# wendongbi/Bridged-GNN

Hardware: AMD Instinct MI355X
Metric: aggregated_edges_per_sec_ktgnn_fwd (higher is better)
Workload: dtype f32; 1 GPU; C4 synthetic bridged graph (local) N=1000000 E'=20991058, 2-layer KT-GNN eval fwd F=128 hidden=128 C=2; parallelism=single, execution=eager launches

## Files before the change

### bridged_gnn_amd/_lib.py

```python
import ctypes as C
import os

import torch

_HERE = os.path.dirname(os.path.abspath(__file__))
SO_PATH = os.path.join(_HERE, "csrc", "libbgnn_hip.so")
_lib = None

_P, _I64, _I32, _F32, _SZ, _INT = C.c_void_p, C.c_int64, C.c_int32, C.c_float, C.c_size_t, C.c_int

SIGNATURES = {
    "bgnn_version": (_INT, []),
    "bgnn_source_hash": (C.c_char_p, []),
    "bgnn_error_string": (C.c_char_p, [_INT]),
    "bgnn_csr_workspace_bytes": (_SZ, [_I64, _I64]),
    "bgnn_build_dst_csr": (_INT, [_P, _I64, _I64, _INT, _P, _P, _P, _P, _P, _SZ, _P]),
    "bgnn_domain_sums_f64": (_INT, [_P, _I64, _I32, _I64, _P, _P, _P]),
    "bgnn_domain_sums_workspace_bytes": (_SZ, [_I32]),
    "bgnn_domain_sums_ws_f64": (_INT, [_P, _I64, _I32, _I64, _P, _P, _P, _SZ, _P]),
    "bgnn_domain_delta_f32": (_INT, [_P, _I32, _P, _P]),
    "bgnn_adaptedconv_transform_f32": (_INT, [_P, _I64, _I32, _I64, _P, _P, _I32, _I32, _P, _P, _P, _P,
                                               _P, _P, _P, _P, _I64, _I64, _P, _P]),
    "bgnn_adaptedconv_transform_sums_f32": (_INT, [_P, _I64, _I32, _I64, _P, _P, _I32, _I32, _P, _P, _P, _P,
                                                    _P, _P, _P, _P, _I64, _I64, _I64, _I64, _P, _P]),
    "bgnn_adaptedconv_transform_need_f32": (_INT, [_P, _I64, _I32, _I64, _P, _P, _I32, _I32, _P, _P, _P, _P,
                                                    _P, _P, _P, _P, _I64, _I64, _P, _P, _P]),
    "bgnn_classifier_stage_f32": (_INT, [_P, _I64, _I32, _I64, _P, _P, _I32, _I32, _P, _P, _P, _P, _P, _P, _P, _P, _I64, _I64,
                                          _P, _P, _I32, _INT, _P, _P, _P, _P, _P, _P]),
    "bgnn_linear_narrow_transform_f32": (_INT, [_P, _I64, _I32, _I64, _P, _P, _I32, _INT, _P, _P, _P, _P, _P, _P]),
    "bgnn_narrow_transform_finish_f32": (_INT, [_P, _I64, _P, _P, _I32, _P, _P, _P, _P, _P, _P, _I64, _P, _P]),
    "bgnn_gram_workspace_bytes": (C.c_size_t, [_I32, _I32]),
    "bgnn_gram_f32": (_INT, [_P, _I64, _I32, _P, _I64, _I32, _I64, _P, _P, C.c_size_t, _P]),
    "bgnn_transform_bwd_prep_workspace_bytes": (C.c_size_t, [_I64, _I32]),
    "bgnn_transform_bwd_prep_f32": (_INT, [_P, _I64, _I64, _I32, _P, _P, _I64, _I32, _P, _P, _P, _P, _P, _P, _I32, _I64, _P, _I64, _P, _P, C.c_size_t, _P]),
    "bgnn_bn_acc_doubles": (_I64, [_I32]),
    "bgnn_bn_relu_dropout_f32": (_INT, [_P, _I64, _I32, _I64, _P, _P, _F32, _INT, _F32, C.c_uint64, _P, _F32, _P, _P, _P, _I64, _P, _P]),
    "bgnn_bn_relu_dropout_bwd_f32": (_INT, [_P, _P, _I64, _I32, _I64, _I64, _P, _P, _P, _F32, _INT, _F32, C.c_uint64, _P, _P, _I64, _P, _P]),
    "bgnn_bn_colstats_f32": (_INT, [_P, _I64, _I32, _I64, _P, _P]),
    "bgnn_bn_apply_rows_f32": (_INT, [_P, _I64, _I32, _I64, _P, _I64, _P, _P, _F32, _INT, _F32, C.c_uint64, _P, _P, _I64, _F32, _P, _P, _P, _I64, _P]),
    "bgnn_bn_bwd_reduce_rows_f32": (_INT, [_P, _P, _I64, _I32, _I64, _I64, _P, _I64, _P, _P, _F32, _INT, _F32, C.c_uint64, _P, _P, _I64, _P, _P]),
    "bgnn_bn_bwd_apply_rows_f32": (_INT, [_P, _P, _I64, _I32, _I64, _I64, _P, _P, _I64, _P, _P, _F32, _INT, _F32, C.c_uint64, _P, _P, _I64, _P, _I64, _P]),
    "bgnn_transform_bwd_consts_f32": (_INT, [_P, _P, _P, _P, _P, _I32, _I32, _P, _P, _P, _P]),
    "bgnn_transform_bwd_finish_f32": (_INT, [_P, _P, _P, _P, _P, _P, _P, _I32, _I32, _I32, _P, _P, _P, _P, _P, _P, _P, _I64, _P]),
    "bgnn_rowdot_f32": (_INT, [_P, _I64, _I64, _I32, _P, _I64, _I32, _P, _P]),
    "bgnn_linear_f32": (_INT, [_P, _I64, _I32, _I64, _P, _P, _I32, _INT, _P, _P, _P, _I64, _P]),
    "bgnn_adaptedconv_aggregate_f32": (_INT, [_P, _P, _I64, _P, _P, _P, _P, _P, _I64, _I64, _I32, _F32,
                                               _P, _I64, _P, _P, _P, _INT, _P, _INT, _I64, _I32, _P, _P, _P]),
    "bgnn_adaptedconv_aggregate_bounded_f32": (_INT, [_P, _P, _I64, _P, _P, _P, _P, _P, _I64, _I64, _I32, _F32,
                                                       _P, _I64, _P, _P, _P, _INT, _P, _INT, _I64, _I32, _P, _P, _I64, _I32, _P]),
    "bgnn_aggregate_hub_workspace_bytes": (C.c_size_t, [_I64, _I32, _I64]),
    "bgnn_adaptedconv_aggregate_hub_f32": (_INT, [_P, _P, _I64, _P, _P, _P, _P, _P, _I64, _I32, _F32, _P, _I64, _P, _P, _INT, _P, _I32, _P,
                                                   _P, _I32, _P, _I64, _P, _P, _P, _I64, _P, _P, C.c_size_t, _P]),
    "bgnn_adaptedconv_aggregate_bwd_f32": (_INT, [_P, _P, _I64, _P, _P, _P, _P, _P, _I64, _I64, _I32, _F32,
                                                   _P, _I64, _P, _P, _I64, _P, _P, _P, _P, _P]),
    "bgnn_aggregate_bwd_pull_workspace_bytes": (C.c_size_t, [_I64, _I64, _I64]),
    "bgnn_adaptedconv_aggregate_bwd_pull_f32": (_INT, [_P, _P, _I64, _P, _P, _P, _P, _P, _P, _P, _P, _I64, _I64, _I32, _F32,
                                                        _P, _I64, _P, _P, _I64, _P, _P, _P, _P, _P, C.c_size_t, _P]),
    "bgnn_aggregate_bwd_pull_hub_workspace_bytes": (C.c_size_t, [_I64, _I64, _I64, _I64, _I64]),
    "bgnn_adaptedconv_aggregate_bwd_pull_hub_f32": (_INT, [_P, _P, _I64, _P, _P, _P, _P, _P, _P, _P, _P, _I64, _I64, _I32, _F32,
                                                            _P, _I64, _P, _P, _I64, _P, _P, _P, _P, _I32,
                                                            _P, _I64, _P, _P, _P, _I64, _P, _I64, _P, _P, _P, _I64, _P, C.c_size_t, _P]),
    "bgnn_aggregate_heads_bwd_workspace_bytes": (C.c_size_t, [_I64, _I64, _I32]),
    "bgnn_adaptedconv_aggregate_heads_bwd_f32": (_INT, [_P, _P, _P, _P, _P, _P, _P, _P, _P, _P, _I64, _I64, _I32, _I32, _F32,
                                                         _P, _P, _P, _INT, _P, _P, _P, _P, _P, C.c_size_t, _P]),
    "bgnn_aggregate_heads_bwd_hub_workspace_bytes": (C.c_size_t, [_I64, _I64, _I32, _I64, _I64]),
    "bgnn_adaptedconv_aggregate_heads_bwd_hub_f32": (_INT, [_P, _P, _P, _P, _P, _P, _P, _P, _P, _I64, _I64, _I32, _I32, _F32,
                                                             _P, _P, _P, _INT, _P, _P, _P, _P, _I32,
                                                             _P, _I64, _P, _P, _P, _I64, _P, _I64, _P, _P, _P, _I64, _P, C.c_size_t, _P]),
    "bgnn_adaptedconv_aggregate_heads_wide_f32": (_INT, [_P, _P, _I64, _P, _P, _P, _P, _P, _I64, _I32, _I32, _F32, _P, _P, _P]),
    "bgnn_aggregate_heads_wide_bwd_workspace_bytes": (C.c_size_t, [_I64, _I32, _I64]),
    "bgnn_adaptedconv_aggregate_heads_wide_bwd_f32": (_INT, [_P, _P, _I64, _P, _P, _P, _P, _P, _P, _P, _I64, _I32, _I32, _F32,
                                                              _P, _P, _P, _P, _P, _P, _P, _P, C.c_size_t, _P]),
    "bgnn_l2_normalize_rows_f32": (_INT, [_P, _I64, _I32, _F32, _P, _P]),
    "bgnn_topk_workspace_bytes": (_SZ, [_I64, _I64, _I32]),
    "bgnn_cosine_topk_f32": (_INT, [_P, _P, _I64, _I64, _I32, _I32, _INT, _P, _P, _P, _P, _SZ, _P]),
    "bgnn_mlp_pair_topk_f32": (_INT, [_P, _P, _P, _P, _P, _F32, _I64, _I64, _I32, _I32, _INT, _P, _P, _P,
                                       _P, _SZ, _P]),
    "bgnn_topk_edges_i64": (_INT, [_P, _I64, _I32, _I64, _I64, _P, _P]),
    "bgnn_topk_edges_coalesced_workspace_bytes": (_SZ, [_I64, _I32]),
    "bgnn_topk_edges_coalesced_i64": (_INT, [_P, _I64, _I32, _I64, _I64, _I64, _P, _P, _SZ, _P]),
    "bgnn_gather_rows_f32": (_INT, [_P, _I64, _I64, _P, _I64, _I32, _P, _I64, _P]),
    "bgnn_coalesce_workspace_bytes": (_SZ, [_I64]),
    "bgnn_coalesce_i64": (_INT, [_P, _I64, _I64, _P, _P, _SZ, _P]),
    "bgnn_sage_mean_aggregate_f32": (_INT, [_P, _I64, _I64, _P, _I64, _P, _P, _I64, _I32, _INT, _INT, _F32, C.c_uint64, _P,
                                             _P, _I64, _P]),
    "bgnn_sage_mean_aggregate_rows_f32": (_INT, [_P, _I64, _I64, _P, _I64, _P, _P, _I64, _I32, _INT, _INT, _F32, C.c_uint64, _P,
                                                  _P, _P, _I64, _P]),
    "bgnn_rows_segment_add_f32": (_INT, [_P, _I64, _I64, _P, _P, _P, _I64, _I32, _INT, _P, _I64, _I64, _P]),
    "bgnn_pair_mlp_workspace_bytes": (_SZ, [_I64]),
    "bgnn_pair_mlp_stats_f32": (_INT, [_P, _I64, _I64, _P, _I64, _I64, _P, _P, _I64, _F32, _P, _P, _P, _P, _SZ, _P]),
    "bgnn_pair_mlp_loss_f32": (_INT, [_P, _I64, _I64, _P, _I64, _I64, _P, _P, _P, _I64, _P, _P, _P, _P, _P, _F32, _P, _P, _P, _P,
                                       _SZ, _P]),
    "bgnn_pair_mlp_segsum_f32": (_INT, [_P, _I64, _I64, _P, _I64, _I64, _P, _P, _P, _I64, _P, _P, _P, _P, _P, _P, _F32, _P, _I64, _P]),
    "bgnn_pair_mlp_eval_f32": (_INT, [_P, _I64, _I64, _P, _I64, _I64, _P, _P, _P, _I64, _P, _P, _P, _P, _P, _P, _P, _SZ, _P]),
    "bgnn_pair_mlp_count_workspace_bytes": (_SZ, [_I64, _I64]),
    "bgnn_pair_mlp_count_f32": (_INT, [_P, _I64, _I64, _P, _I64, _I64, _P, _I64, _P, _I64, _P, _P, _P, _P, _P, _P, _P, _P, _SZ, _P]),
    "bgnn_pair_cos_loss_workspace_bytes": (_SZ, [_I64]),
    "bgnn_pair_cos_count_workspace_bytes": (_SZ, [_I64, _I64]),
    "bgnn_pair_cos_loss_f32": (_INT, [_P, _I64, _I64, _P, _I64, _I64, _P, _P, _P, _I64, _P, _P, _P, _P, _SZ, _P]),
    "bgnn_pair_cos_segsum_f32": (_INT, [_P, _I64, _I64, _P, _P, _P, _I64, _P, _I64, _P, _I64, _P]),
    "bgnn_pair_cos_count_f32": (_INT, [_P, _I64, _I64, _P, _I64, _I64, _P, _I64, _P, _I64, _P, _P, _P, _P, _SZ, _P]),
    "bgnn_sage_mean_aggregate_bwd_workspace_bytes": (_SZ, [_I64, _I32]),
    "bgnn_sage_mean_aggregate_bwd_f32": (_INT, [_P, _I64, _P, _I64, _P, _I64, _P, _P, _I64, _I32, _INT, _F32, _P, _I64, _P, _I64,
                                                 _P, _SZ, _P]),
    "bgnn_gcn_aggregate_workspace_bytes": (_SZ, [_I64, _I32]),
    "bgnn_gcn_aggregate_f32": (_INT, [_P, _I64, _I64, _P, _P, _P, _P, _I64, _I64, _I32, _INT, _F32, C.c_uint64, _P,
                                       _I32, _P, _I64, _P, _P, _I64, _P, _SZ, _P, _I64, _P]),
    "bgnn_gcn_aggregate_rows_f32": (_INT, [_P, _I64, _I64, _P, _P, _P, _P, _I64, _I64, _I32, _INT, _F32, C.c_uint64, _P,
                                            _I32, _P, _I64, _P, _P, _I64, _P, _SZ, _P, _P, _I64, _P]),
    "bgnn_gcn_aggregate_bwd_f32": (_INT, [_P, _I64, _P, _I64, _I64, _P, _P, _P, _I64, _I64, _I32, _INT, _F32,
                                           _I32, _P, _I64, _P, _P, _I64, _P, _SZ, _P, _I64, _P, _I64, _P]),
    "bgnn_step2_loss_workspace_bytes": (_SZ, [_I64, _I32]),
    "bgnn_step2_loss_f32": (_INT, [_P, _I64, _P, _I64, _P, _I64, _I64, _I32, _P, _P, _P, C.c_double, _P, _P, _SZ, _P]),
    "bgnn_step2_loss_bwd_f32": (_INT, [_P, _I64, _P, _I64, _I64, _I32, _P, _P, _P, C.c_double, _P, _P, _P, _P, _P, _I64, _P]),
    "bgnn_step2_nll_f32": (_INT, [_P, _I64, _I64, _I32, _P, _P, _P, _P, _SZ, _P]),
    "bgnn_step2_nll_bwd_f32": (_INT, [_I64, _I32, _P, _P, _P, _P, _P, _I64, _P]),
    "bgnn_step2_counts_f32": (_INT, [_P, _I64, _P, _I64, _P, _I64, _I64, _I32, _P, _P, C.c_uint64, _I32, _P, _P]),
    "bgnn_step2_auc_count_f32": (_INT, [_P, _P, _I64, _P, _P, _P, _P]),
    "bgnn_adam_chunk_elems": (_I64, []),
    "bgnn_adam_step_f32": (_INT, [_P, _I32, _P, _I64, _P, _P, _I64, C.c_double, C.c_double, C.c_double, C.c_double, _P]),
    "bgnn_quantile_workspace_bytes": (_SZ, [_I64]),
    "bgnn_quantile_f32": (_INT, [_P, _I64, C.c_double, _P, _P, _SZ, _P]),
    "bgnn_row_inv_norms_f32": (_INT, [_P, _I64, _I32, _F32, _P, _P]),
    "bgnn_edge_validity_f32": (_INT, [_P, _I64, _P, _I64, _P, _P, _P, _P, _I64, _P, _P, _P, _P, _I32, _INT, _F32, _P, _P, _I32, _P, _P, _P, _P]),
    "bgnn_edge_rule1_counts_f32": (_INT, [_P, _P, _I64, _P, _P, _P]),
}


def source_hash():
    import hashlib
    csrc = os.path.join(_HERE, "csrc")
    h = hashlib.sha256()
    for name in _HASHED_SOURCES:
        with open(os.path.join(csrc, name), "rb") as f:
            h.update(f.read())
    return h.hexdigest()[:16]


_HASHED_SOURCES = ("bgnn_api.hip", "bgnn_csr.hip", "bgnn_transform.hip", "bgnn_transform_stream.hip", "bgnn_transform_cls.hip", "bgnn_aggregate.hip", "bgnn_aggregate_bwd.hip",
                   "bgnn_aggregate_bwd_fast.hip", "bgnn_knn.hip", "bgnn_gram.hip", "bgnn_norm.hip", "bgnn_sage.hip", "bgnn_gcn.hip", "bgnn_aggregate_heads_wide.hip", "bgnn_pair_mlp.hip", "bgnn_pair_cos.hip", "bgnn_step2.hip", "bgnn_optim.hip", "bgnn_edge_filter.hip", "bgnn_common.h", "bgnn_transform_params.h", "bgnn_aggregate_bwd_params.h", os.path.join("..", "..", "include", "bgnn.h"))


def _sidecar_hash():
    try:
        with open(os.path.join(_HERE, "csrc", "libbgnn_hip.srchash")) as f:
            return f.read().strip()
    except OSError:
        return None


ABI_VERSION = 113


def _make():
    import fcntl
    import subprocess
    csrc = os.path.join(_HERE, "csrc")
    with open(os.path.join(csrc, ".build.lock"), "w") as lock:
        fcntl.flock(lock, fcntl.LOCK_EX)
        try:
            if os.path.exists(SO_PATH) and _sidecar_hash() == source_hash():
                return
            r = subprocess.run(["make", "-C", csrc, "-j4", "-s"], stdout=subprocess.PIPE, stderr=subprocess.STDOUT, text=True)
            if r.returncode != 0:
                raise RuntimeError(f"building {SO_PATH} failed (make exit code {r.returncode}):\n{r.stdout[-4000:]}")
        finally:
            fcntl.flock(lock, fcntl.LOCK_UN)


def _load():
    l = C.CDLL(SO_PATH)
    for name, (res, args) in SIGNATURES.items():
        fn = getattr(l, name)
        fn.restype, fn.argtypes = res, args
    return l


def lib():
    global _lib
    if _lib is None:
        have_hipcc = os.path.exists("/opt/rocm/bin/hipcc")
        if have_hipcc and (not os.path.exists(SO_PATH) or _sidecar_hash() != source_hash()):
            _make()
        if not os.path.exists(SO_PATH):
            raise RuntimeError(
                f"{SO_PATH} is missing: build it with `python -c 'import __graft_entry__ as g; g.build()'` "
                "(or `make -C bridged_gnn_amd/csrc`).  bridged_gnn_amd has no CPU fallback.")
        want = source_hash()
        l = _load()
        got = l.bgnn_source_hash().decode()
        if got != want:
            raise RuntimeError(
                f"{SO_PATH} was built from other sources (library {got}, tree {want}): rebuild it with "
                "`make -C bridged_gnn_amd/csrc` (a loaded library cannot be replaced inside this process)")
        if l.bgnn_version() != ABI_VERSION:
            raise RuntimeError(f"{SO_PATH} exports ABI revision {l.bgnn_version()}, this binding was written for {ABI_VERSION}")
        _lib = l
    return _lib


def check(rc, what):
    if rc != 0:
        msg = lib().bgnn_error_string(int(rc))
# ... 37 lines not shown
```

### bridged_gnn_amd/classifier_stage.py

```python
import os

import torch
import torch.nn.functional as F

from . import ops
from .ktgnn import _AggregateFn, _AggregateHeadsFn, _AggregateWideHeadsFn, _TransformPairFn, _pad_cols4, _plist


class ClassifierStage:

    def __init__(self, model):
        base = model.clf_base
        self.model, self.convs = model, (base, model.clf_target, model.clf_target)
        self.C, self.ld, self.slope = base.out_channels, ops.pad4(base.out_channels), base.negative_slope
        self.plain = not (base.root_weight or base.normalize)
        self.fused_log_softmax = ops.heads_log_softmax_supported(3, self.C)
        self.drop_caches()

    def drop_caches(self):
        self._a3_key = self._tf_key = self._tf_pack = None

    def views(self, t2s, s2t):
        ld = self.ld
        return [(t2s[:, j * ld:(j + 1) * ld], s2t[:, j * ld:(j + 1) * ld]) for j in range(3)]

    def attention(self, autograd=False):
        if autograd:
            return (torch.stack([c.a_f_t2s.weight.reshape(-1) for c in self.convs]),
                    torch.stack([c.a_f_s2t.weight.reshape(-1) for c in self.convs]))
        key = (self.convs[0]._versions(), self.convs[1]._versions())
        if self._a3_key != key:
            self._a3 = (torch.stack([c.a_f_t2s.weight.detach().reshape(-1) for c in self.convs]).contiguous(),
                        torch.stack([c.a_f_s2t.weight.detach().reshape(-1) for c in self.convs]).contiguous())
            self._a3_key = key
        return self._a3

    def finish(self, out3):
        logp = out3.view(out3.shape[0], 3, self.ld)[:, :, :self.C]
        if not self.fused_log_softmax:
            logp = F.log_softmax(logp, dim=2)
        return logp[:, 0], logp[:, 1], logp[:, 2]

    def fold_transformer(self):
        l0, bn, _, l3 = self.model.clf_transformer
        key = tuple((p.data_ptr(), p._version) for p in _plist(self.model.clf_transformer)) + \
            (bn.running_mean._version, bn.running_var._version)
        if self._tf_key != key:
            s = (bn.weight / torch.sqrt(bn.running_var + bn.eps)).detach()
            self._tf_w0 = (l0.weight.detach() * s[:, None]).float().contiguous()
            self._tf_w0t = self._tf_w0.t().contiguous()
            self._tf_b0 = (l0.bias.detach() * s + bn.bias.detach() - bn.running_mean * s).float().contiguous()
            self._tf_key = key
            self._tf_pack = None

    def transformer_hidden_eval(self, x, mask_u8=None, want_sums=False, sums_out=None):
        self.fold_transformer()
        sums = None
        dout, din = self._tf_w0.shape
        if x.dtype == torch.float32 and x.stride(1) == 1 and ops.linear_supported(din, dout):
            if want_sums:
                sums = sums_out if sums_out is not None else torch.zeros(2 * dout + 2, dtype=torch.float64, device=x.device)
            h1 = ops.linear(x, self._tf_w0, self._tf_b0, relu=True, mask_u8=mask_u8 if want_sums else None, colsum=sums)
        elif hasattr(torch, "_addmm_activation"):
            h1 = torch._addmm_activation(self._tf_b0, x, self._tf_w0t, use_gelu=False)
        else:
            h1 = F.relu(torch.addmm(self._tf_b0, x, self._tf_w0t))
        return (h1, sums) if want_sums else h1

    def transformer_eval(self, x):
        l3 = self.model.clf_transformer[3]
        return F.linear(self.transformer_hidden_eval(x), l3.weight, l3.bias)

    def composed_target_pack(self, din_pad):
        c, l3 = self.convs[1], self.model.clf_transformer[3]
        key = (din_pad, c._versions(), l3.weight._version, l3.bias._version, l3.weight.data_ptr())
        if self._tf_pack is None or self._tf_pack[0] != key:
            W3, b3 = l3.weight.detach(), l3.bias.detach()
            hd = c.head()
            din = W3.shape[0]

            def comp_gate(g):
                g = g.reshape(-1)
                return torch.cat((W3.t() @ g[:din], W3.t() @ g[din:])), (b3 * g[:din]).sum()
            g1, c1 = comp_gate(hd["g_s2t"])
            g2, c2 = comp_gate(hd["g_t2s"])
            head = {"W_s": hd["W_s"] @ W3, "W_t": hd["W_t"] @ W3,
                    "b_s": hd["W_s"] @ b3 + (hd["b_s"] if hd["b_s"] is not None else 0),
                    "b_t": hd["W_t"] @ b3 + (hd["b_t"] if hd["b_t"] is not None else 0),
                    "g_s2t": g1, "g_t2s": g2, "gate_const": (c1, c2)}
            self._tf_pack = (key, ops.pack_transform_heads([head], din_pad))
        return self._tf_pack[1]

    def one_pass(self, x, mask_u8, sums_h, views, arena):
        if sums_h is None or x.dtype != torch.float32 or x.stride(1) != 1:
            return None
        self.fold_transformer()
        dout, din = self._tf_w0.shape
        if x.shape[1] != din or dout != 128:
            return None
        pack_t = self.composed_target_pack(ops.pad4(dout))
        pair = self.convs[0].packed(x.shape[1], self.convs[1])
        if not ops.classifier_stage_supported(x, pair, self._tf_w0, pack_t):
            return None
        n_s = 2 * ops.pad4(dout) + 2
        sums_t = arena.take(n_s) if arena is not None else torch.zeros(n_s, dtype=torch.float64, device=x.device)
        raw = ops.classifier_stage(x, mask_u8, sums_h, pair, [views[0], views[1]], self._tf_w0, self._tf_b0, sums_t, pack_t, relu=True)
        return raw, None, sums_t

    def pair_tables(self, x, mask_u8, sums_h, views):
        self.convs[0].transform(x, mask_u8, sums=sums_h, partner=self.convs[1], out=[views[0], views[1]])

    def target_stage_a(self, x, mask_u8, sums_out=None):
        self.fold_transformer()
        dout, din = self._tf_w0.shape
        pack = self.composed_target_pack(ops.pad4(dout))
        if (sums_out is not None and x.dtype == torch.float32 and x.stride(1) == 1 and x.shape[1] == din
                and ops.linear_narrow_supported(din, dout, pack) and os.environ.get("BGNN_FUSED_TARGET", "1") != "0"):
            return ops.linear_narrow_transform(x, self._tf_w0, self._tf_b0, mask_u8, sums_out, pack, relu=True), None, sums_out
        h1, sums1 = self.transformer_hidden_eval(x, mask_u8, want_sums=True, sums_out=sums_out)
        h1 = _pad_cols4(h1)
        if sums1 is None or sums1.numel() != 2 * h1.shape[1] + 2:
            sums1 = ops.domain_sums(h1, mask_u8)
        return None, h1, sums1

    def target_stage_b(self, stage_a, mask_u8, out, sums_t=None):
        raw, h1, sums_t = (*stage_a[:2], sums_t if sums_t is not None else stage_a[2])
        if raw is not None:
            ops.narrow_transform_finish(raw, mask_u8, sums_t, self.composed_target_pack(ops.pad4(self._tf_w0.shape[0])), out)
        else:
            ops.adaptedconv_transform(h1, mask_u8, None, self.composed_target_pack(h1.shape[1]), out=[out], sums=sums_t)

    def target_tables(self, x, mask_u8, out, arena=None, sums_out=None):
        if sums_out is None:
            n_s = 2 * ops.pad4(self.model.clf_transformer[0].weight.shape[0]) + 2
            sums_out = arena.take(n_s) if arena is not None else torch.zeros(n_s, dtype=torch.float64, device=x.device)
        self.target_stage_b(self.target_stage_a(x, mask_u8, sums_out), mask_u8, out)

    def eval_tables(self, x, mask_u8, sums_h, views, arena):
        a = self.one_pass(x, mask_u8, sums_h, views, arena)
        if a is not None:
            return self.target_stage_b(a, mask_u8, views[2])
        self.pair_tables(x, mask_u8, sums_h, views)
        self.target_tables(x, mask_u8, views[2], arena)

    def train_walk(self, opt_in=False):
        if ops.heads_log_softmax_supported(3, self.C) and not (opt_in and os.environ.get("BGNN_FUSED_TRAIN_HEADS", "1") == "0"):
            return "narrow"
        if ops.wide_heads_supported(3, self.C) and not (opt_in and os.environ.get("BGNN_WIDE_TRAIN_HEADS", "0") != "1"):
            return "wide"
        return None if opt_in else "convs"

    def train_tables(self, x, mask_u8, sums_x, bn, sums_of=None, mean_hook=None):
        base, target, _ = self.convs
        l0, bnm, _, l3 = self.model.clf_transformer
        xt = l3(bn(l0(x), bnm, True, 0.0)).contiguous()
        sums_t = sums_of(xt) if sums_of is not None else None
        if mean_hook is None and _TransformPairFn.supported(x, base, target):
            prm = [t for c in (base, target)
                   for t in (c.lin_s.weight, c.lin_s.bias, c.lin_t.weight, c.lin_t.bias, c.a_g_s2t.weight, c.a_g_t2s.weight)]
            tabs_x = _TransformPairFn.apply(x, mask_u8, base, target, sums_x, *prm)
        else:
            tabs_x = (*base._transform_autograd(x, mask_u8, sums_x, mean_hook), *target._transform_autograd(x, mask_u8, sums_x, mean_hook))
        return (*tabs_x, *target._transform_autograd(xt, mask_u8, sums_t, mean_hook))

    def train_aggregate(self, walk, csr, mask_u8, tables, n_rows=None):
        C = self.C
        a_t, a_s = self.attention(autograd=True)
        if walk == "convs":
            return tuple(F.log_softmax(_AggregateFn.apply(tables[2 * j], tables[2 * j + 1], a_t[j], a_s[j], csr, mask_u8, C,
                                                          c.negative_slope)[:n_rows, :C], dim=1) for j, c in enumerate(self.convs))
        fn = _AggregateHeadsFn if walk == "narrow" else _AggregateWideHeadsFn
        logp = fn.apply(csr, mask_u8, C, self.slope, a_t, a_s, *tables)[:n_rows, :, :C]
        return logp[:, 0], logp[:, 1], logp[:, 2]
```

### bridged_gnn_amd/csrc/bgnn_aggregate.hip

```cpp
#include <cstdlib>
#include "bgnn_common.h"

namespace {

struct AggParams {
  const float* h_t2s;
  const float* h_s2t;
  int64_t ldh;
  const float* a_t2s;
  const float* a_s2t;
  const int32_t* rowptr;
  const int32_t* col;
  const uint8_t* mask;
  int64_t row_begin;
  int64_t row_end;
  int32_t D;
  float slope;
  float* out;
  int64_t ldo;
  float* alpha;
  const float* ep_scale;
  const float* ep_shift;
  int ep_relu;
  unsigned int* tile_queue;
  double* colsum;
  int32_t heads;
  float* state_ms;
  int mode;
  int64_t park_begin;
  int tq_chunk;
  int tq_interleave;
  int xcd_segments;
  const int32_t* vrow_node;
  const int32_t* vrow_bounds;
  int64_t n_vrows;
  float* vout; float* vms;
  int32_t hub_threshold;
  const char* tbl_base;
  uint32_t tbl_bytes, off_t2s, off_s2t;
  int32_t gather_hint;
  uint32_t dead_off;
};

__device__ __forceinline__ float leaky(float v, float slope) { return v > 0.f ? v : v * slope; }

template <int LF, int EP, int U>
__global__ __launch_bounds__(256) void agg_kernel(AggParams p) {
  constexpr int GL = LF * EP;
  constexpr int GPW = 64 / GL;
  constexpr int RPB = 4 * GPW;
  const int lane = threadIdx.x & 63;
  const int wave = threadIdx.x >> 6;
  const int g = lane / GL;
  const int lg = lane % GL;
  const int sub = lg / LF;
  const int f0 = (lg % LF) * 4;
  const bool fvalid = f0 < p.D;

  const int64_t ntiles = ((p.row_end - p.row_begin) * p.heads + RPB - 1) / RPB;
  bgnn::XcdRange tr = bgnn::xcd_pos_range(ntiles);
  __shared__ float red[2][LF * 4 + 1];
  if (p.colsum != nullptr) {
    for (int t = threadIdx.x; t < 2 * (LF * 4 + 1); t += 256) (&red[0][0])[t] = 0.f;
    __syncthreads();
  }

  __shared__ unsigned int dyn_tile;
  const int64_t xbase = tr.begin - (blockIdx.x / 8);
  int64_t tile = tr.begin - tr.step;
  int64_t chunk_left = 0;
  const int TQ_CHUNK = p.tq_chunk;
  for (;;) {
    if (p.tile_queue != nullptr) {
      if (chunk_left == 0) {
        __syncthreads();
        if (threadIdx.x == 0) dyn_tile = atomicAdd(&p.tile_queue[blockIdx.x % 8], 1u);
        __syncthreads();
        tile = xbase + (int64_t)dyn_tile * TQ_CHUNK;
        chunk_left = TQ_CHUNK;
      } else {
        tile += 1;
      }
      --chunk_left;
    } else {
      tile += tr.step;
    }
    if (tile >= tr.end) break;
    const int64_t gt = bgnn::xcd_tile_of(tile, ntiles);
    if (gt < 0) continue;
    const int64_t i = p.row_begin * p.heads + gt * RPB + wave * GPW + g;
    const bool rvalid = i < p.row_end * p.heads;
    const int64_t ic = rvalid ? i : p.row_begin * p.heads;
    const int64_t node = ic / p.heads;
    const int head = (int)(ic - node * p.heads);
    const bool dom_s = p.mask[node] != 0;
    const float* __restrict__ H = dom_s ? p.h_t2s : p.h_s2t;
    const float* __restrict__ av = (dom_s ? p.a_t2s : p.a_s2t) + head * p.D;
    const int32_t beg = rvalid ? p.rowptr[node] : 0;
    const int32_t end = rvalid ? p.rowptr[node + 1] : 0;

    float4 a4 = make_float4(0.f, 0.f, 0.f, 0.f), hi = a4;
    if (fvalid) {
      a4.x = av[f0];
      a4.y = f0 + 1 < p.D ? av[f0 + 1] : 0.f;
      a4.z = f0 + 2 < p.D ? av[f0 + 2] : 0.f;
      a4.w = f0 + 3 < p.D ? av[f0 + 3] : 0.f;
      hi = *reinterpret_cast<const float4*>(H + ic * p.ldh + f0);
    }

    float m = -INFINITY, s = 0.f;
    float4 acc = make_float4(0.f, 0.f, 0.f, 0.f);
    if (p.mode == 2 && rvalid && sub == 0) {
      m = p.state_ms[2 * i];
      s = p.state_ms[2 * i + 1];
      if (f0 < p.ldo) acc = *reinterpret_cast<const float4*>(p.out + i * p.ldo + f0);
    }
    const int32_t deg = end - beg;
    const int32_t niter = (deg + EP * U - 1) / (EP * U);

    int32_t nid[U];
#pragma unroll
    for (int u = 0; u < U; ++u) {
      int32_t e = beg + sub + u * EP;
      nid[u] = e < end ? p.col[e] : -1;
    }
    for (int32_t it = 0; it < niter; ++it) {
      const int32_t e0 = beg + it * (EP * U) + sub;
      int32_t id[U];
      float4 v[U];
#pragma unroll
      for (int u = 0; u < U; ++u) {
        id[u] = nid[u];
        v[u] = make_float4(0.f, 0.f, 0.f, 0.f);
        if (id[u] >= 0 && fvalid) v[u] = *reinterpret_cast<const float4*>(H + ((int64_t)id[u] * p.heads + head) * p.ldh + f0);
      }
#pragma unroll
      for (int u = 0; u < U; ++u) {
        int32_t e = e0 + (U + u) * EP;
        nid[u] = e < end ? p.col[e] : -1;
      }
      float lg_[U];
      float cm = -INFINITY;
#pragma unroll
      for (int u = 0; u < U; ++u) {
        float t = a4.x * leaky(v[u].x + hi.x, p.slope);
        t = fmaf(a4.y, leaky(v[u].y + hi.y, p.slope), t);
        t = fmaf(a4.z, leaky(v[u].z + hi.z, p.slope), t);
        t = fmaf(a4.w, leaky(v[u].w + hi.w, p.slope), t);
        t = bgnn::group_sum<LF>(t);
        lg_[u] = id[u] >= 0 ? t : -INFINITY;
        cm = fmaxf(cm, lg_[u]);
      }
      if (p.alpha != nullptr && (lg % LF) == 0) {
#pragma unroll
        for (int u = 0; u < U; ++u)
          if (id[u] >= 0) p.alpha[e0 + u * EP] = lg_[u];
      }
      const float mn = fmaxf(m, cm);
      const float sc = (m == mn) ? 1.f : __expf(m - mn);
      s *= sc;
      acc.x *= sc; acc.y *= sc; acc.z *= sc; acc.w *= sc;
#pragma unroll
      for (int u = 0; u < U; ++u) {
        const float pe = (lg_[u] == -INFINITY) ? 0.f : __expf(lg_[u] - mn);
        s += pe;
        acc.x = fmaf(pe, v[u].x, acc.x);
        acc.y = fmaf(pe, v[u].y, acc.y);
        acc.z = fmaf(pe, v[u].z, acc.z);
        acc.w = fmaf(pe, v[u].w, acc.w);
      }
      m = mn;
    }

#pragma unroll
    for (int off = LF; off < GL; off <<= 1) {
      const float m2 = __shfl_xor(m, off);
      const float s2 = __shfl_xor(s, off);
      float4 b;
      b.x = __shfl_xor(acc.x, off); b.y = __shfl_xor(acc.y, off);
      b.z = __shfl_xor(acc.z, off); b.w = __shfl_xor(acc.w, off);
      const float mn = fmaxf(m, m2);
      const float c1 = (m == mn) ? 1.f : __expf(m - mn);
      const float c2 = (m2 == mn) ? 1.f : __expf(m2 - mn);
      s = s * c1 + s2 * c2;
      acc.x = acc.x * c1 + b.x * c2; acc.y = acc.y * c1 + b.y * c2;
      acc.z = acc.z * c1 + b.z * c2; acc.w = acc.w * c1 + b.w * c2;
      m = mn;
    }

    if (p.mode == 1 && node >= p.park_begin) {
      if (rvalid && sub == 0) {
        if (lg == 0) { p.state_ms[2 * i] = m; p.state_ms[2 * i + 1] = s; }
        if (f0 < p.ldo) *reinterpret_cast<float4*>(p.out + i * p.ldo + f0) = fvalid ? acc : make_float4(0.f, 0.f, 0.f, 0.f);
      }
// ... 406 lines not shown
      const int32_t j = tile - xbase, sg = j / seg_len;
      gt = (sg * 8 + xcd) * seg_len + (j - sg * seg_len);
      if (gt >= ntiles) continue;
    }
    const int32_t i0 = row0 + gt * RPB + wave * GPW + g;
    const bool rvalid = i0 < row1;
    const int32_t ic = rvalid ? i0 : row0;
    const bool dom_s = p.mask[ic] != 0;
    const int32_t beg = rvalid ? p.rowptr[ic] : 0;
    const int32_t end = rvalid ? p.rowptr[ic + 1] : 0;
    const uint32_t lbase = (dom_s ? p.off_t2s : p.off_s2t) + (uint32_t)f0c * 4u;
    const f2 a01 = dom_s ? aS01 : aT01, a23 = dom_s ? aS23 : aT23;
    const float4 hi4 = __builtin_bit_cast(float4, __builtin_amdgcn_raw_buffer_load_b128(rt, lbase + __umul24((uint32_t)ic, nstride), 0, 0));
    f2 h01 = {hi4.x, hi4.y}, h23 = {hi4.z, hi4.w};

    float m = -INFINITY, s = 0.f;
    f2 acc01 = {0.f, 0.f}, acc23 = {0.f, 0.f};
    const int32_t niter = (end - beg + U - 1) / U;
    auto issue = [&](float4 (&v)[U], uint32_t off) {
      v[0] = __builtin_bit_cast(float4, __builtin_amdgcn_raw_buffer_load_b128(rt, lbase + dpp_movu<0x00>(off), 0, 0));
      v[1] = __builtin_bit_cast(float4, __builtin_amdgcn_raw_buffer_load_b128(rt, lbase + dpp_movu<0x55>(off), 0, 0));
      v[2] = __builtin_bit_cast(float4, __builtin_amdgcn_raw_buffer_load_b128(rt, lbase + dpp_movu<0xAA>(off), 0, 0));
      v[3] = __builtin_bit_cast(float4, __builtin_amdgcn_raw_buffer_load_b128(rt, lbase + dpp_movu<0xFF>(off), 0, 0));
      asm volatile("" : "+v"(h01), "+v"(h23) : : "memory");
      __builtin_amdgcn_sched_barrier(0);
    };
    auto take_id = [&](uint32_t& id) {
      __builtin_amdgcn_sched_barrier(0);
      asm volatile("s_waitcnt vmcnt(0)" : "+v"(id), "+v"(m), "+v"(s), "+v"(acc01), "+v"(acc23) : : "memory");
    };
    auto load_id = [&](int32_t ee) {
      uint32_t id;
      const uint32_t eoff = (uint32_t)max(min(ee, end - 1), 0) * 4u;
      __builtin_amdgcn_sched_barrier(0);
      asm volatile("global_load_dword %0, %1, %2" : "=v"(id) : "v"(eoff), "s"(p.col) : "memory");
      __builtin_amdgcn_sched_barrier(0);
      return id;
    };
    auto row_off = [&](uint32_t id, bool alive) { return alive ? __umul24(id, nstride) : p.dead_off; };
    auto update = [&](const float4 (&v)[U], bool ok, int32_t e_cur) {
      float t[U];
#pragma unroll
      for (int u = 0; u < U; ++u) {
        f2 z0 = f2{v[u].x, v[u].y} + h01, z1 = f2{v[u].z, v[u].w} + h23;
        z0 = __builtin_elementwise_max(z0, z0 * sl);
        z1 = __builtin_elementwise_max(z1, z1 * sl);
        f2 q = a01 * z0;
        q = __builtin_elementwise_fma(a23, z1, q);
        t[u] = q.x + q.y;
      }
      const float rA = bfly<0xB1>(b0, t[0], t[1]), rB = bfly<0xB1>(b0, t[2], t[3]);
      float r = bfly<0x4E>(b1, rA, rB);
      r += bgnn::dpp_mov<0x124>(r);
      r += bgnn::dpp_mov<0x128>(r);
      if constexpr (LF >= 32) r += bgnn::swz_xor16(r);
      if constexpr (LF >= 64) r += __shfl_xor(r, 32);
      const float l = ok ? r : -INFINITY;
      if constexpr (ALPHA) {
        if (lg < U && ok) p.alpha[e_cur] = l;
      }
      float cm = fmaxf(l, bgnn::dpp_mov<0xB1>(l));
      cm = fmaxf(cm, bgnn::dpp_mov<0x4E>(cm));
      const float mn = fmaxf(m, cm);
      const float sc = (m == mn) ? 1.f : __expf(m - mn);
      const float pe = (l == -INFINITY) ? 0.f : __expf(l - mn);
      s = fmaf(s, sc, pe);
      const f2 sc2 = {sc, sc};
      acc01 *= sc2; acc23 *= sc2;
#define BGNN_ACC(u, w)                                               \
      {                                                              \
        acc01.x = fmaf(w, v[u].x, acc01.x); acc01.y = fmaf(w, v[u].y, acc01.y); \
        acc23.x = fmaf(w, v[u].z, acc23.x); acc23.y = fmaf(w, v[u].w, acc23.y); \
      }
#ifdef AGGF_X_NOACC
      acc01.x += pe * v[0].x + v[1].y + v[2].z + v[3].w;
#else
      { const float w = quad_bcast<0>(pe); BGNN_ACC(0, w) }
      { const float w = quad_bcast<1>(pe); BGNN_ACC(1, w) }
      { const float w = quad_bcast<2>(pe); BGNN_ACC(2, w) }
      { const float w = quad_bcast<3>(pe); BGNN_ACC(3, w) }
#endif
#undef BGNN_ACC
      m = mn;
    };
    int32_t nw = __builtin_amdgcn_readlane(niter, 0);
    if constexpr (LF <= 32) nw = max(nw, __builtin_amdgcn_readlane(niter, 32));
    if constexpr (LF <= 16) nw = max(nw, max(__builtin_amdgcn_readlane(niter, 16), __builtin_amdgcn_readlane(niter, 48)));
    int32_t e = beg + k;
    bool ok = e < end;
    uint32_t myoff = p.dead_off;
    if (nw > 0) myoff = row_off((uint32_t)p.col[max(min(e, end - 1), 0)], ok);
    for (int32_t it = 0; it < nw; ++it) {
      float4 v[U];
      issue(v, myoff);
      const int32_t e_cur = e;
      e += U;
      const bool ok2 = e < end;
      uint32_t nextid = load_id(e);
      update(v, ok, e_cur);
      ok = ok2;
      take_id(nextid);
      myoff = row_off(nextid, ok);
    }
    s += bgnn::dpp_mov<0xB1>(s);
    s += bgnn::dpp_mov<0x4E>(s);

    const float inv = 1.f / (s + 1e-16f);
    if constexpr (ALPHA) {
      if (lg < U) {
        for (int32_t e2 = beg + lg; e2 < end; e2 += 4 * U) {
          float a[4];
#pragma unroll
          for (int j = 0; j < 4; ++j) a[j] = e2 + j * U < end ? p.alpha[e2 + j * U] : 0.f;
#pragma unroll
          for (int j = 0; j < 4; ++j)
            if (e2 + j * U < end) p.alpha[e2 + j * U] = __expf(a[j] - m) * inv;
        }
      }
    }
    if (rvalid && f0 < p.ldo) {
      float4 o = make_float4(acc01.x * inv, acc01.y * inv, acc23.x * inv, acc23.y * inv);
      if (p.ep_scale != nullptr) {
        o.x = fmaf(o.x, sc4[0], sh4[0]); o.y = fmaf(o.y, sc4[1], sh4[1]);
        o.z = fmaf(o.z, sc4[2], sh4[2]); o.w = fmaf(o.w, sc4[3], sh4[3]);
      }
      if (p.ep_relu) { o.x = fmaxf(o.x, 0.f); o.y = fmaxf(o.y, 0.f); o.z = fmaxf(o.z, 0.f); o.w = fmaxf(o.w, 0.f); }
      if (!fvalid) o = make_float4(0.f, 0.f, 0.f, 0.f);
      __builtin_amdgcn_raw_buffer_store_b128(__builtin_bit_cast(u32x4_t, o), ro, __umul24((uint32_t)i0, ostride) + (uint32_t)f0 * 4u, 0, 0);
      if (p.colsum != nullptr) {
        const float ws = dom_s ? 1.f : 0.f, wt = dom_s ? 0.f : 1.f;
        const f2 ws2 = {ws, ws}, wt2 = {wt, wt}, o01 = {o.x, o.y}, o23 = {o.z, o.w};
        cs_s01 = __builtin_elementwise_fma(o01, ws2, cs_s01); cs_s23 = __builtin_elementwise_fma(o23, ws2, cs_s23);
        cs_t01 = __builtin_elementwise_fma(o01, wt2, cs_t01); cs_t23 = __builtin_elementwise_fma(o23, wt2, cs_t23);
        n_s += ws; n_t += wt;
      }
    }
  }
  if (p.colsum != nullptr) {
    unsafeAtomicAdd(&red[0][f0], cs_s01.x); unsafeAtomicAdd(&red[0][f0 + 1], cs_s01.y);
    unsafeAtomicAdd(&red[0][f0 + 2], cs_s23.x); unsafeAtomicAdd(&red[0][f0 + 3], cs_s23.y);
    unsafeAtomicAdd(&red[1][f0], cs_t01.x); unsafeAtomicAdd(&red[1][f0 + 1], cs_t01.y);
    unsafeAtomicAdd(&red[1][f0 + 2], cs_t23.x); unsafeAtomicAdd(&red[1][f0 + 3], cs_t23.y);
    if (lg == 0) { unsafeAtomicAdd(&red[0][LF * 4], n_s); unsafeAtomicAdd(&red[1][LF * 4], n_t); }
    __syncthreads();
    for (int t = threadIdx.x; t < 2 * (LF * 4 + 1); t += 256) {
      const int d = t / (LF * 4 + 1), c = t % (LF * 4 + 1);
      const double sum = (double)red[d][c];
      if (c == LF * 4) unsafeAtomicAdd(&p.colsum[2 * p.ldo + d], sum);
      else if (c < p.ldo) unsafeAtomicAdd(&p.colsum[d * p.ldo + c], sum);
    }
  }
}

template <int HEADS, int EP, int U>
__global__ __launch_bounds__(256) void agg_heads_lanes_kernel(AggParams p) {
  constexpr int GL = EP * HEADS, GPW = 64 / GL, RPB = 4 * GPW;
  const int lane = threadIdx.x & 63, wave = threadIdx.x >> 6;
  const int g = lane / GL, lg = lane % GL;
  const int sub = lg / HEADS, h = lg % HEADS;
  const bool lane_on = g < GPW;
  const int64_t ntiles = (p.row_end - p.row_begin + p.n_vrows + RPB - 1) / RPB;
  bgnn::XcdRange tr = bgnn::xcd_pos_range(ntiles);
  const int64_t rs = (int64_t)HEADS * p.ldh;
  for (int64_t pos = tr.begin; pos < tr.end; pos += tr.step) {
    const int64_t tile = bgnn::xcd_tile_of(pos, ntiles);
    if (tile < 0) continue;
    const int64_t i = p.row_begin + tile * RPB + wave * GPW + g;
    const bool in_range = lane_on && i < p.row_end + p.n_vrows;
    const bool virt = in_range && i >= p.row_end;
    const int64_t vix = virt ? i - p.row_end : 0;
    const int64_t ic = in_range ? i : p.row_begin;
    const int64_t node = virt ? (int64_t)p.vrow_node[vix] : ic;
    const bool dom_s = p.mask[node] != 0;
    const float* __restrict__ H = dom_s ? p.h_t2s : p.h_s2t;
    const float* __restrict__ av = dom_s ? p.a_t2s : p.a_s2t;
    int32_t beg = in_range ? (virt ? p.vrow_bounds[2 * vix] : p.rowptr[ic]) : 0;
    int32_t end = in_range ? (virt ? p.vrow_bounds[2 * vix + 1] : p.rowptr[ic + 1]) : 0;
    const bool hub = !virt && p.hub_threshold > 0 && end - beg >= p.hub_threshold;
    const bool rvalid = in_range && !hub;
    const int64_t oi = virt ? vix : i;
    float* __restrict__ obase = virt ? p.vout : p.out;
    float* __restrict__ msbase = virt ? p.vms : p.state_ms;
    if (hub) { beg = 0; end = 0; }
    float4 a4;
    a4.x = av[h * p.D];
    a4.y = p.D > 1 ? av[h * p.D + 1] : 0.f;
    a4.z = p.D > 2 ? av[h * p.D + 2] : 0.f;
    a4.w = p.D > 3 ? av[h * p.D + 3] : 0.f;
    const float4 hi = *reinterpret_cast<const float4*>(H + node * rs + h * p.ldh);
    float4 acc = make_float4(0.f, 0.f, 0.f, 0.f);
    float m = -INFINITY, s = 0.f;
    if (p.mode == 2 && rvalid && !virt && sub == 0) {
      m = p.state_ms[2 * (i * HEADS + h)];
      s = p.state_ms[2 * (i * HEADS + h) + 1];
      acc = *reinterpret_cast<const float4*>(p.out + (i * HEADS + h) * p.ldo);
    }
    const int32_t niter = (end - beg + EP * U - 1) / (EP * U);
    for (int32_t it = 0; it < niter; ++it) {
      int32_t id[U];
      float4 v[U];
#pragma unroll
      for (int u = 0; u < U; ++u) {
        const int32_t e = beg + it * (EP * U) + sub + u * EP;
        id[u] = e < end ? p.col[e] : -1;
      }
#pragma unroll
      for (int u = 0; u < U; ++u)
        v[u] = id[u] >= 0 ? *reinterpret_cast<const float4*>(H + (int64_t)id[u] * rs + h * p.ldh) : make_float4(0.f, 0.f, 0.f, 0.f);
      float lg_[U], cm = -INFINITY;
#pragma unroll
      for (int u = 0; u < U; ++u) {
        float t = a4.x * leaky(v[u].x + hi.x, p.slope);
        t = fmaf(a4.y, leaky(v[u].y + hi.y, p.slope), t);
        t = fmaf(a4.z, leaky(v[u].z + hi.z, p.slope), t);
        t = fmaf(a4.w, leaky(v[u].w + hi.w, p.slope), t);
        lg_[u] = id[u] >= 0 ? t : -INFINITY;
        cm = fmaxf(cm, lg_[u]);
      }
      const float mn = fmaxf(m, cm);
      const float sc = (m == mn) ? 1.f : __expf(m - mn);
      s *= sc;
      acc.x *= sc; acc.y *= sc; acc.z *= sc; acc.w *= sc;
#pragma unroll
      for (int u = 0; u < U; ++u) {
        const float pe = (lg_[u] == -INFINITY) ? 0.f : __expf(lg_[u] - mn);
        s += pe;
        acc.x = fmaf(pe, v[u].x, acc.x); acc.y = fmaf(pe, v[u].y, acc.y);
        acc.z = fmaf(pe, v[u].z, acc.z); acc.w = fmaf(pe, v[u].w, acc.w);
      }
      m = mn;
    }
#pragma unroll
    for (int off = 1; off < EP; off <<= 1) {
      const int src = (sub ^ off) * HEADS + h + g * GL;
      const int from = lane_on ? src : lane;
      const float m2 = __shfl(m, from), s2 = __shfl(s, from);
      float4 b;
      b.x = __shfl(acc.x, from); b.y = __shfl(acc.y, from); b.z = __shfl(acc.z, from); b.w = __shfl(acc.w, from);
      const float mn = fmaxf(m, m2);
      const float c1 = (m == mn) ? 1.f : __expf(m - mn), c2 = (m2 == mn) ? 1.f : __expf(m2 - mn);
      s = s * c1 + s2 * c2;
      acc.x = acc.x * c1 + b.x * c2; acc.y = acc.y * c1 + b.y * c2;
      acc.z = acc.z * c1 + b.z * c2; acc.w = acc.w * c1 + b.w * c2;
      m = mn;
    }
    if (rvalid && sub == 0) {
      float* o = obase + (oi * HEADS + h) * p.ldo;
      if (virt || (p.mode == 1 && i >= p.park_begin)) {
        msbase[2 * (oi * HEADS + h)] = m;
        msbase[2 * (oi * HEADS + h) + 1] = s;
        *reinterpret_cast<float4*>(o) = acc;
      } else {
        const float inv = 1.f / (s + 1e-16f);
        float4 r = make_float4(acc.x * inv, acc.y * inv, acc.z * inv, acc.w * inv);
        if (p.mode == 3) {
          p.state_ms[2 * (i * HEADS + h)] = m;
          p.state_ms[2 * (i * HEADS + h) + 1] = s;
        }
        if (p.ep_relu == 2) {
          float mx = r.x;
          if (p.D > 1) mx = fmaxf(mx, r.y);
          if (p.D > 2) mx = fmaxf(mx, r.z);
          if (p.D > 3) mx = fmaxf(mx, r.w);
          float se = expf(r.x - mx);
          if (p.D > 1) se += expf(r.y - mx);
          if (p.D > 2) se += expf(r.z - mx);
          if (p.D > 3) se += expf(r.w - mx);
          const float lse = logf(se);
          r.x = r.x - mx - lse;
          r.y = p.D > 1 ? r.y - mx - lse : 0.f;
          r.z = p.D > 2 ? r.z - mx - lse : 0.f;
          r.w = p.D > 3 ? r.w - mx - lse : 0.f;
        }
        *reinterpret_cast<float4*>(o) = r;
      }
    }
  }
}

inline int tq_chunk_for(int64_t ntiles, int64_t grid) {
  static const int forced = [] { const char* e = getenv("BGNN_AGG_CHUNK"); return e ? atoi(e) : 0; }();
  (void)ntiles; (void)grid;
  return forced > 0 ? forced : 4;
}

template <int HEADS, int EP, int U>
int launch_heads(const AggParams& p, hipStream_t st) {
  constexpr int RPB = 4 * (64 / (EP * HEADS));
  static const int cap = [] {
    int per_cu = 0, dev = 0;
    hipDeviceProp_t prop;
    if (hipGetDevice(&dev) != hipSuccess || hipGetDeviceProperties(&prop, dev) != hipSuccess) return 2048;
    if (hipOccupancyMaxActiveBlocksPerMultiprocessor(&per_cu, agg_heads_lanes_kernel<HEADS, EP, U>, 256, 0) != hipSuccess || per_cu < 1) return 2048;
    if (per_cu > 8) per_cu = 8;
    return per_cu * prop.multiProcessorCount / 8 * 8;
  }();
  const int64_t ntiles = (p.row_end - p.row_begin + p.n_vrows + RPB - 1) / RPB;
  int64_t grid = ntiles < cap ? (ntiles + 7) / 8 * 8 : cap;
  if (grid < 8) grid = 8;
  hipLaunchKernelGGL((agg_heads_lanes_kernel<HEADS, EP, U>), dim3((unsigned)grid), dim3(256), 0, st, p);
  BGNN_LAUNCH_CHECK();
  return 0;
}

template <int LF, int EP, int U>
int resident_blocks() {
  static const int nb = [] {
    int per_cu = 0, dev = 0;
    hipDeviceProp_t prop;
    if (hipGetDevice(&dev) != hipSuccess || hipGetDeviceProperties(&prop, dev) != hipSuccess) return 2048;
    if (hipOccupancyMaxActiveBlocksPerMultiprocessor(&per_cu, agg_kernel<LF, EP, U>, 256, 0) != hipSuccess || per_cu < 1)
      return 2048;
    if (per_cu > 8) per_cu = 8;
    return per_cu * prop.multiProcessorCount / 8 * 8;
  }();
  return nb;
}

template <int LF, int EP, int U>
int launch(const AggParams& p, hipStream_t st) {
  constexpr int RPB = 4 * (64 / (LF * EP));
  int64_t ntiles = ((p.row_end - p.row_begin) * p.heads + RPB - 1) / RPB;
  const int64_t cap = resident_blocks<LF, EP, U>();
  int64_t grid = ntiles < cap ? (ntiles + 7) / 8 * 8 : cap;
  if (grid < 8) grid = 8;
  AggParams q = p;
  q.tq_chunk = tq_chunk_for(ntiles, grid);
  hipLaunchKernelGGL((agg_kernel<LF, EP, U>), dim3((unsigned)grid), dim3(256), 0, st, q);
  BGNN_LAUNCH_CHECK();
  return 0;
}

template <int LF, int U>
int launch_wide(const AggParams& p, hipStream_t st) {
  constexpr int RPB = 4 * (64 / LF);
  static const int cap = [] {
    int per_cu = 0, dev = 0;
    hipDeviceProp_t prop;
    if (hipGetDevice(&dev) != hipSuccess || hipGetDeviceProperties(&prop, dev) != hipSuccess) return 2048;
    if (hipOccupancyMaxActiveBlocksPerMultiprocessor(&per_cu, agg_wide_kernel<LF, U>, 256, 0) != hipSuccess || per_cu < 1) return 2048;
    if (per_cu > 8) per_cu = 8;
    const char* e = getenv("BGNN_AGG_BLOCKS_PER_CU");
    if (e && atoi(e) > 0 && atoi(e) < per_cu) per_cu = atoi(e);
    return per_cu * prop.multiProcessorCount / 8 * 8;
  }();
  const int64_t ntiles = ((p.row_end - p.row_begin) * p.heads + p.n_vrows + RPB - 1) / RPB;
  int64_t grid = ntiles < cap ? (ntiles + 7) / 8 * 8 : cap;
  if (grid < 8) grid = 8;
  AggParams q = p;
  q.tq_chunk = tq_chunk_for(ntiles, grid);
  static const int il = [] { const char* e = getenv("BGNN_AGG_INTERLEAVE"); return e ? atoi(e) : 1; }();
  q.tq_interleave = il;
  static const int nseg = [] { const char* e = getenv("BGNN_XCD_SEGMENTS"); return e ? atoi(e) : 8; }();
  q.xcd_segments = nseg;
  hipLaunchKernelGGL((agg_wide_kernel<LF, U>), dim3((unsigned)grid), dim3(256), 0, st, q);
  BGNN_LAUNCH_CHECK();
  return 0;
}

static bool fast_plan(AggParams& p, int64_t table_rows) {
  static const bool on = [] { const char* e = getenv("BGNN_AGG_FAST"); return !(e && atoi(e) == 0); }();
  if (!on || table_rows <= 0) return false;
  if (p.heads != 1 || p.mode != 0 || p.n_vrows != 0 || p.hub_threshold != 0) return false;
  const int64_t lim24 = (int64_t)1 << 24, lim32 = ((int64_t)1 << 32) - 1;
  if (table_rows > lim24 || p.row_end > table_rows || p.ldh * 4 >= lim24 || p.ldo * 4 >= lim24) return false;
  const char* a = reinterpret_cast<const char*>(p.h_t2s);
  const char* b = reinterpret_cast<const char*>(p.h_s2t);
  const char* lo = a < b ? a : b;
  const int64_t span = (int64_t)((a < b ? b : a) - lo) + table_rows * p.ldh * 4;
  if (span > lim32 || p.row_end * p.ldo * 4 > lim32) return false;
  p.tbl_base = lo;
  p.tbl_bytes = (uint32_t)span;
  p.off_t2s = (uint32_t)(a - lo);
  p.off_s2t = (uint32_t)(b - lo);
  const int64_t lane_max = (span - table_rows * p.ldh * 4) + p.ldh * 4, dead = (((int64_t)1 << 32) - 16) - lane_max;
  p.dead_off = dead >= span ? (uint32_t)dead : 0u;
  return true;
}

template <int LF, bool ALPHA>
int launch_wide_fast(const AggParams& p, hipStream_t st) {
  constexpr int RPB = 4 * (64 / LF);
  static const int per_cu_max = [] {
    int per_cu = 0;
    if (hipOccupancyMaxActiveBlocksPerMultiprocessor(&per_cu, agg_wide_fast_kernel<LF, ALPHA>, 256, 0) != hipSuccess || per_cu < 1) return 0;
    if (per_cu > 8) per_cu = 8;
    const char* e = getenv("BGNN_AGG_BLOCKS_PER_CU");
    if (e && atoi(e) > 0 && atoi(e) < per_cu) per_cu = atoi(e);
    return per_cu;
  }();
  static const int n_cu = [] {
    int dev = 0;
    hipDeviceProp_t prop;
    if (hipGetDevice(&dev) != hipSuccess || hipGetDeviceProperties(&prop, dev) != hipSuccess) return 0;
    return prop.multiProcessorCount;
  }();
  static const bool forced = getenv("BGNN_AGG_BLOCKS_PER_CU") != nullptr;
  int per_cu = per_cu_max;
  if (p.gather_hint == 2 && !forced && per_cu > 3) per_cu = 3;
  const int64_t cap = (per_cu_max > 0 && n_cu > 0) ? (int64_t)per_cu * n_cu / 8 * 8 : 2048;
  const int64_t ntiles = (p.row_end - p.row_begin + RPB - 1) / RPB;
  int64_t grid = ntiles < cap ? (ntiles + 7) / 8 * 8 : cap;
  if (grid < 8) grid = 8;
  AggParams q = p;
  q.tq_chunk = tq_chunk_for(ntiles, grid);
  static const int il = [] { const char* e = getenv("BGNN_AGG_INTERLEAVE"); return e ? atoi(e) : 1; }();
  q.tq_interleave = il;
  static const int nseg = [] { const char* e = getenv("BGNN_XCD_SEGMENTS"); return e ? atoi(e) : 8; }();
  q.xcd_segments = nseg;
  hipLaunchKernelGGL((agg_wide_fast_kernel<LF, ALPHA>), dim3((unsigned)grid), dim3(256), 0, st, q);
  BGNN_LAUNCH_CHECK();
  return 0;
}

struct HubMergeParams {
  const int32_t* hub_rows; const int32_t* seg_ptr; int64_t n_hubs;
  const float* part_acc;
  const float* part_ms;
  const uint8_t* mask;
  int32_t D; int64_t ldo; int32_t heads;
  float* out; const float* ep_scale; const float* ep_shift; int ep_relu;
  double* colsum; float* state_ms;
  float* alpha; const int32_t* rowptr;
};

template <int LF>
__global__ __launch_bounds__(256) void hub_merge_wide_kernel(HubMergeParams p) {
  const int lane = threadIdx.x % LF, grp = threadIdx.x / LF;
  constexpr int GPB = 256 / LF;
  const int f0 = lane * 4;
  const bool fvalid = f0 < p.D;
  __shared__ float red[2][LF * 4 + 1];
  if (p.colsum != nullptr) {
    for (int t = threadIdx.x; t < 2 * (LF * 4 + 1); t += 256) (&red[0][0])[t] = 0.f;
    __syncthreads();
  }
  float sc4[4] = {1.f, 1.f, 1.f, 1.f}, sh4[4] = {0.f, 0.f, 0.f, 0.f};
  if (p.ep_scale != nullptr) {
#pragma unroll
    for (int c = 0; c < 4; ++c)
      if (f0 + c < p.D) { sc4[c] = p.ep_scale[f0 + c]; sh4[c] = p.ep_shift[f0 + c]; }
  }
  float4 cs_s = make_float4(0.f, 0.f, 0.f, 0.f), cs_t = cs_s;
  float n_s = 0.f, n_t = 0.f;
  for (int64_t hrow = (int64_t)blockIdx.x * GPB + grp; hrow < p.n_hubs; hrow += (int64_t)gridDim.x * GPB) {
    const int64_t node = p.hub_rows[hrow];
    float m = -INFINITY, s = 0.f;
    float4 acc = make_float4(0.f, 0.f, 0.f, 0.f);
    const int32_t v1 = p.seg_ptr[hrow + 1];
    for (int32_t v0 = p.seg_ptr[hrow]; v0 < v1; v0 += 4) {
      float m2[4], s2[4];
      float4 b[4];
#pragma unroll
      for (int u = 0; u < 4; ++u) {
        const int64_t v = v0 + u < v1 ? v0 + u : v1 - 1;
        m2[u] = v0 + u < v1 ? p.part_ms[2 * v] : -INFINITY;
        s2[u] = v0 + u < v1 ? p.part_ms[2 * v + 1] : 0.f;
        b[u] = f0 < p.ldo ? *reinterpret_cast<const float4*>(p.part_acc + v * p.ldo + f0) : make_float4(0.f, 0.f, 0.f, 0.f);
      }
#pragma unroll
      for (int u = 0; u < 4; ++u) {
        const float mn = fmaxf(m, m2[u]);
        const float c1 = (m == mn) ? 1.f : __expf(m - mn), c2 = (m2[u] == mn) ? 1.f : __expf(m2[u] - mn);
        s = s * c1 + s2[u] * c2;
        acc.x = acc.x * c1 + b[u].x * c2; acc.y = acc.y * c1 + b[u].y * c2;
        acc.z = acc.z * c1 + b[u].z * c2; acc.w = acc.w * c1 + b[u].w * c2;
        m = mn;
      }
    }
    if (p.alpha != nullptr) {
      const float inv = 1.f / (s + 1e-16f);
      for (int32_t e = p.rowptr[node] + lane; e < p.rowptr[node + 1]; e += LF) p.alpha[e] = __expf(p.alpha[e] - m) * inv;
    }
    if (f0 < p.ldo) {
      const float inv = 1.f / (s + 1e-16f);
      float4 o = make_float4(acc.x * inv, acc.y * inv, acc.z * inv, acc.w * inv);
      if (p.ep_scale != nullptr) {
        o.x = fmaf(o.x, sc4[0], sh4[0]); o.y = fmaf(o.y, sc4[1], sh4[1]);
        o.z = fmaf(o.z, sc4[2], sh4[2]); o.w = fmaf(o.w, sc4[3], sh4[3]);
      }
      if (p.ep_relu) { o.x = fmaxf(o.x, 0.f); o.y = fmaxf(o.y, 0.f); o.z = fmaxf(o.z, 0.f); o.w = fmaxf(o.w, 0.f); }
      if (!fvalid) o = make_float4(0.f, 0.f, 0.f, 0.f);
      *reinterpret_cast<float4*>(p.out + node * p.ldo + f0) = o;
      if (p.mask[node] != 0) { cs_s.x += o.x; cs_s.y += o.y; cs_s.z += o.z; cs_s.w += o.w; n_s += 1.f; }
      else                   { cs_t.x += o.x; cs_t.y += o.y; cs_t.z += o.z; cs_t.w += o.w; n_t += 1.f; }
    }
  }
  if (p.colsum != nullptr) {
    unsafeAtomicAdd(&red[0][f0], cs_s.x); unsafeAtomicAdd(&red[0][f0 + 1], cs_s.y);
    unsafeAtomicAdd(&red[0][f0 + 2], cs_s.z); unsafeAtomicAdd(&red[0][f0 + 3], cs_s.w);
    unsafeAtomicAdd(&red[1][f0], cs_t.x); unsafeAtomicAdd(&red[1][f0 + 1], cs_t.y);
    unsafeAtomicAdd(&red[1][f0 + 2], cs_t.z); unsafeAtomicAdd(&red[1][f0 + 3], cs_t.w);
    if (lane == 0) { unsafeAtomicAdd(&red[0][LF * 4], n_s); unsafeAtomicAdd(&red[1][LF * 4], n_t); }
    __syncthreads();
    for (int t = threadIdx.x; t < 2 * (LF * 4 + 1); t += 256) {
      const int d = t / (LF * 4 + 1), c = t % (LF * 4 + 1);
      const double sum = (double)red[d][c];
      if (c == LF * 4) unsafeAtomicAdd(&p.colsum[2 * p.ldo + d], sum);
      else if (c < p.ldo) unsafeAtomicAdd(&p.colsum[d * p.ldo + c], sum);
    }
  }
}

__global__ __launch_bounds__(256) void hub_merge_heads_kernel(HubMergeParams p) {
  const int64_t t = (int64_t)blockIdx.x * 256 + threadIdx.x;
  if (t >= p.n_hubs * p.heads) return;
  const int64_t hrow = t / p.heads;
  const int h = (int)(t - hrow * p.heads);
  const int64_t node = p.hub_rows[hrow];
  float m = -INFINITY, s = 0.f;
  float4 acc = make_float4(0.f, 0.f, 0.f, 0.f);
  for (int32_t v = p.seg_ptr[hrow]; v < p.seg_ptr[hrow + 1]; ++v) {
    const int64_t e = (int64_t)v * p.heads + h;
    const float m2 = p.part_ms[2 * e], s2 = p.part_ms[2 * e + 1];
    const float4 b = *reinterpret_cast<const float4*>(p.part_acc + e * p.ldo);
    const float mn = fmaxf(m, m2);
    const float c1 = (m == mn) ? 1.f : __expf(m - mn), c2 = (m2 == mn) ? 1.f : __expf(m2 - mn);
    s = s * c1 + s2 * c2;
    acc.x = acc.x * c1 + b.x * c2; acc.y = acc.y * c1 + b.y * c2;
    acc.z = acc.z * c1 + b.z * c2; acc.w = acc.w * c1 + b.w * c2;
    m = mn;
  }
  const float inv = 1.f / (s + 1e-16f);
  float4 r = make_float4(acc.x * inv, acc.y * inv, acc.z * inv, acc.w * inv);
  if (p.state_ms != nullptr) {
    p.state_ms[2 * (node * p.heads + h)] = m;
    p.state_ms[2 * (node * p.heads + h) + 1] = s;
  }
  if (p.ep_relu == 2) {
    float mx = r.x;
    if (p.D > 1) mx = fmaxf(mx, r.y);
    if (p.D > 2) mx = fmaxf(mx, r.z);
    if (p.D > 3) mx = fmaxf(mx, r.w);
    float se = expf(r.x - mx);
    if (p.D > 1) se += expf(r.y - mx);
    if (p.D > 2) se += expf(r.z - mx);
    if (p.D > 3) se += expf(r.w - mx);
    const float lse = logf(se);
    r.x = r.x - mx - lse;
    r.y = p.D > 1 ? r.y - mx - lse : 0.f;
    r.z = p.D > 2 ? r.z - mx - lse : 0.f;
    r.w = p.D > 3 ? r.w - mx - lse : 0.f;
  }
  *reinterpret_cast<float4*>(p.out + (node * p.heads + h) * p.ldo) = r;
}

static int dispatch_aggregate(const AggParams& p, hipStream_t st, int64_t table_rows = 0) {
  const int32_t D = p.D, heads = p.heads;
  if (heads == 3 && D <= 4 && p.ldh == 4 && p.ldo == 4) return launch_heads<3, 2, 4>(p, st);
  if (heads == 2 && D <= 4 && p.ldh == 4 && p.ldo == 4) return launch_heads<2, 2, 4>(p, st);
  const int nv = (D + 3) / 4;
  if (nv <= 1) return launch<1, 4, 4>(p, st);
  if (nv <= 2) return launch<2, 2, 4>(p, st);
  if (nv <= 4) return launch<4, 1, 8>(p, st);
  if (nv <= 8) return launch<8, 1, 4>(p, st);
  const bool wide_ok = p.slope >= 0.f && p.slope <= 1.f && (int64_t)heads * p.ldh * 4 < (int64_t)1 << 32;
  if (wide_ok) {
    AggParams q = p;
    if (fast_plan(q, table_rows)) {
      if (q.alpha != nullptr) {
        if (nv <= 16) return launch_wide_fast<16, true>(q, st);
        if (nv <= 32) return launch_wide_fast<32, true>(q, st);
        return launch_wide_fast<64, true>(q, st);
      }
      if (nv <= 16) return launch_wide_fast<16, false>(q, st);
      if (nv <= 32) return launch_wide_fast<32, false>(q, st);
      return launch_wide_fast<64, false>(q, st);
    }
    if (nv <= 16) return launch_wide<16, 4>(p, st);
    if (nv <= 32) return launch_wide<32, 4>(p, st);
    return launch_wide<64, 4>(p, st);
  }
  if (nv <= 16) return launch<16, 1, 8>(p, st);
  if (nv <= 32) return launch<32, 1, 4>(p, st);
  return launch<64, 1, 4>(p, st);
}

static bool hub_capable(int32_t D, int64_t ldh, int64_t ldo, int32_t heads, float slope) {
  if ((heads == 3 || heads == 2) && D <= 4 && ldh == 4 && ldo == 4) return true;
  const int nv = (D + 3) / 4;
  return heads == 1 && nv > 8 && slope >= 0.f && slope <= 1.f && ldh * 4 < (int64_t)1 << 32;
}

}

static int aggregate_impl(const float* h_t2s, const float* h_s2t, int64_t ldh,
                          const float* a_t2s, const float* a_s2t,
                          const int32_t* rowptr, const int32_t* col, const uint8_t* mask,
                          int64_t row_begin, int64_t row_end, int32_t D, float negative_slope,
                          float* out, int64_t ldo, float* alpha_opt,
                          const float* ep_scale_opt, const float* ep_shift_opt, int ep_relu,
                          float* state_ms_opt, int part, int64_t park_begin, int32_t heads,
                          double* colsum_opt, uint32_t* tile_queue_opt, int64_t table_rows, int32_t gather_hint, void* stream) {
  if (colsum_opt && heads != 1) return BGNN_E_SHAPE;
  if (part == 1 && (park_begin < row_begin || park_begin > row_end)) return BGNN_E_SHAPE;
  if (part < 0 || part > 3 || (part != 0 && (!state_ms_opt || alpha_opt))) return BGNN_E_NULL;
  if (part == 3 && !((heads == 3 || heads == 2) && D <= 4 && ldh == 4 && ldo == 4)) return BGNN_E_SHAPE;
  if (heads < 1 || heads > 8 || (heads > 1 && (alpha_opt || ep_scale_opt))) return BGNN_E_SHAPE;
  if (ep_relu < 0 || ep_relu > 2) return BGNN_E_SHAPE;
  if (ep_relu == 2 && !((heads == 3 || heads == 2) && D <= 4 && ldh == 4 && ldo == 4)) return BGNN_E_SHAPE;
  if (!h_t2s || !h_s2t || !a_t2s || !a_s2t || !rowptr || !col || !mask || !out) return BGNN_E_NULL;
  if (row_begin < 0 || row_end < row_begin || D <= 0 || D > 256 || ldh < D || ldo < D) return BGNN_E_SHAPE;
  if ((ldh & 3) || (ldo & 3) || !bgnn_aligned16(h_t2s) || !bgnn_aligned16(h_s2t) || !bgnn_aligned16(out))
    return BGNN_E_ALIGN;
  if ((ep_scale_opt == nullptr) != (ep_shift_opt == nullptr)) return BGNN_E_NULL;
  if (row_end == row_begin) return 0;
  AggParams p{h_t2s, h_s2t, ldh, a_t2s, a_s2t, rowptr, col, mask, row_begin, row_end, D, negative_slope,
              out, ldo, alpha_opt, ep_scale_opt, ep_shift_opt, ep_relu, tile_queue_opt, colsum_opt, heads, state_ms_opt, part,
              park_begin, 4};
  p.gather_hint = gather_hint;
  hipStream_t st = (hipStream_t)stream;
  if (tile_queue_opt) {
    hipError_t e = bgnn_zero_async(tile_queue_opt, 8 * sizeof(uint32_t), st);
    if (e != hipSuccess) return (int)e;
  }
  return dispatch_aggregate(p, st, table_rows);
}

extern "C" int bgnn_adaptedconv_aggregate_f32(const float* h_t2s, const float* h_s2t, int64_t ldh,
                                              const float* a_t2s, const float* a_s2t,
                                              const int32_t* rowptr, const int32_t* col, const uint8_t* mask,
                                              int64_t row_begin, int64_t row_end, int32_t D, float negative_slope,
                                              float* out, int64_t ldo, float* alpha_opt,
                                              const float* ep_scale_opt, const float* ep_shift_opt, int ep_relu,
                                              float* state_ms_opt, int part, int64_t park_begin, int32_t heads,
                                              double* colsum_opt, uint32_t* tile_queue_opt, void* stream) {
  return aggregate_impl(h_t2s, h_s2t, ldh, a_t2s, a_s2t, rowptr, col, mask, row_begin, row_end, D, negative_slope, out, ldo, alpha_opt,
                        ep_scale_opt, ep_shift_opt, ep_relu, state_ms_opt, part, park_begin, heads, colsum_opt, tile_queue_opt, 0, 0, stream);
}

extern "C" int bgnn_adaptedconv_aggregate_bounded_f32(const float* h_t2s, const float* h_s2t, int64_t ldh,
                                                      const float* a_t2s, const float* a_s2t,
                                                      const int32_t* rowptr, const int32_t* col, const uint8_t* mask,
                                                      int64_t row_begin, int64_t row_end, int32_t D, float negative_slope,
                                                      float* out, int64_t ldo, float* alpha_opt,
                                                      const float* ep_scale_opt, const float* ep_shift_opt, int ep_relu,
                                                      float* state_ms_opt, int part, int64_t park_begin, int32_t heads,
                                                      double* colsum_opt, uint32_t* tile_queue_opt, int64_t table_rows, int32_t gather_hint,
                                                      void* stream) {
  if (table_rows < row_end || gather_hint < 0 || gather_hint > 2) return BGNN_E_SHAPE;
  return aggregate_impl(h_t2s, h_s2t, ldh, a_t2s, a_s2t, rowptr, col, mask, row_begin, row_end, D, negative_slope, out, ldo, alpha_opt,
                        ep_scale_opt, ep_shift_opt, ep_relu, state_ms_opt, part, park_begin, heads, colsum_opt, tile_queue_opt, table_rows, gather_hint, stream);
}

extern "C" size_t bgnn_aggregate_hub_workspace_bytes(int64_t n_segments, int32_t heads, int64_t ldo) {
  const size_t nv = (size_t)(n_segments > 0 ? n_segments : 0), h = (size_t)(heads > 0 ? heads : 1);
  return bgnn_align_up(sizeof(float) * nv * h * (size_t)(ldo > 0 ? ldo : 0), 256) + bgnn_align_up(sizeof(float) * 2 * nv * h, 256) + 256;
}

extern "C" int bgnn_adaptedconv_aggregate_hub_f32(const float* h_t2s, const float* h_s2t, int64_t ldh,
                                                  const float* a_t2s, const float* a_s2t,
                                                  const int32_t* rowptr, const int32_t* col, const uint8_t* mask,
                                                  int64_t N, int32_t D, float negative_slope, float* out, int64_t ldo,
                                                  const float* ep_scale_opt, const float* ep_shift_opt, int ep_relu,
                                                  float* state_ms_opt, int32_t heads, double* colsum_opt,
                                                  uint32_t* tile_queue_opt, int32_t hub_threshold, const int32_t* hub_rows,
                                                  int64_t n_hubs, const int32_t* hub_seg_ptr, const int32_t* seg_bounds,
                                                  const int32_t* seg_node, int64_t n_segments, float* alpha_opt,
                                                  void* ws, size_t ws_bytes, void* stream) {
  if (!h_t2s || !h_s2t || !a_t2s || !a_s2t || !rowptr || !col || !mask || !out) return BGNN_E_NULL;
  if (alpha_opt && heads != 1) return BGNN_E_SHAPE;
  if (n_hubs > 0 && (!hub_rows || !hub_seg_ptr || !seg_bounds || !seg_node || !ws)) return BGNN_E_NULL;
  if (N < 0 || D <= 0 || D > 256 || ldh < D || ldo < D || (ldh & 3) || (ldo & 3) || hub_threshold < 2 || n_hubs < 0 || n_segments < n_hubs)
    return BGNN_E_SHAPE;
  if (!hub_capable(D, ldh, ldo, heads, negative_slope)) return BGNN_E_SHAPE;
  if (colsum_opt && heads != 1) return BGNN_E_SHAPE;
  if (heads > 1 && ep_scale_opt) return BGNN_E_SHAPE;
  if (ep_relu < 0 || ep_relu > 2 || (ep_relu == 2 && heads == 1)) return BGNN_E_SHAPE;
  if ((ep_scale_opt == nullptr) != (ep_shift_opt == nullptr)) return BGNN_E_NULL;
  if (!bgnn_aligned16(h_t2s) || !bgnn_aligned16(h_s2t) || !bgnn_aligned16(out) || (ws && !bgnn_aligned16(ws))) return BGNN_E_ALIGN;
  if (n_hubs > 0 && ws_bytes < bgnn_aggregate_hub_workspace_bytes(n_segments, heads, ldo)) return BGNN_E_WORKSPACE;
  if (N == 0) return 0;
  hipStream_t st = (hipStream_t)stream;
  const int part = (state_ms_opt && heads > 1) ? 3 : 0;
  AggParams p{h_t2s, h_s2t, ldh, a_t2s, a_s2t, rowptr, col, mask, 0, N, D, negative_slope,
              out, ldo, alpha_opt, ep_scale_opt, ep_shift_opt, ep_relu, tile_queue_opt, colsum_opt, heads, state_ms_opt, part,
              0, 4};
  p.hub_threshold = n_hubs > 0 ? hub_threshold : 0;
  if (tile_queue_opt) {
    hipError_t e = bgnn_zero_async(tile_queue_opt, 8 * sizeof(uint32_t), st);
    if (e != hipSuccess) return (int)e;
  }
  float* part_acc = n_hubs > 0 ? (float*)ws : nullptr;
  float* part_ms = n_hubs > 0 ? (float*)((char*)ws + bgnn_align_up(sizeof(float) * (size_t)n_segments * (size_t)heads * (size_t)ldo, 256)) : nullptr;
  if (n_hubs > 0) {
    p.vrow_node = seg_node; p.vrow_bounds = seg_bounds; p.n_vrows = n_segments; p.vout = part_acc; p.vms = part_ms;
  }
  int rc = dispatch_aggregate(p, st, N);
  if (rc || n_hubs == 0) return rc;
  HubMergeParams mp{hub_rows, hub_seg_ptr, n_hubs, part_acc, part_ms, mask, D, ldo, heads, out, ep_scale_opt, ep_shift_opt,
                    ep_relu, colsum_opt, part == 3 ? state_ms_opt : nullptr, alpha_opt, rowptr};
  if (heads > 1) {
    hipLaunchKernelGGL(hub_merge_heads_kernel, dim3((unsigned)((n_hubs * heads + 255) / 256)), dim3(256), 0, st, mp);
  } else {
    const int nvs = (D + 3) / 4;
    int64_t grid = n_hubs < 2048 ? n_hubs : 2048;
    if (nvs <= 16) hipLaunchKernelGGL(hub_merge_wide_kernel<16>, dim3((unsigned)((grid + 15) / 16)), dim3(256), 0, st, mp);
    else if (nvs <= 32) hipLaunchKernelGGL(hub_merge_wide_kernel<32>, dim3((unsigned)((grid + 7) / 8)), dim3(256), 0, st, mp);
    else hipLaunchKernelGGL(hub_merge_wide_kernel<64>, dim3((unsigned)((grid + 3) / 4)), dim3(256), 0, st, mp);
  }
  BGNN_LAUNCH_CHECK();
  return 0;
}

#ifdef BGNN_TUNING
extern "C" int bgnn_tune_reset_counters(void* stream) { (void)stream; return 0; }
extern "C" int bgnn_tune_aggregate(const float* h_t2s, const float* h_s2t, int64_t ldh, const float* a_t2s,
                                   const float* a_s2t, const int32_t* rowptr, const int32_t* col, const uint8_t* mask,
                                   int64_t row_begin, int64_t row_end, int32_t D, float slope, float* out, int64_t ldo,
                                   int variant, uint32_t* tile_queue, void* stream) {
  AggParams p{h_t2s, h_s2t, ldh, a_t2s, a_s2t, rowptr, col, mask, row_begin, row_end, D, slope,
              out, ldo, nullptr, nullptr, nullptr, 0, tile_queue, nullptr, 1, nullptr, 0};
  hipStream_t st = (hipStream_t)stream;
  if (tile_queue && bgnn_zero_async(tile_queue, 32, st) != hipSuccess) return -1;
  switch (variant) {
    case 40: return launch_wide<32, 4>(p, st);
    case 41: return launch_wide<32, 8>(p, st);
    case 42: return launch_wide<16, 4>(p, st);
    case 43: return launch_wide<16, 8>(p, st);
    case 44: return launch_wide<64, 4>(p, st);
    case 45: return launch_wide<64, 8>(p, st);
    case 0: return launch<32, 1, 4>(p, st);
    case 1: return launch<32, 1, 8>(p, st);
    case 2: return launch<32, 2, 4>(p, st);
    case 3: return launch<32, 2, 2>(p, st);
    case 4: return launch<32, 1, 2>(p, st);
    case 5: return launch<32, 2, 8>(p, st);
    case 6: return launch<64, 1, 4>(p, st);
    case 10: return launch<1, 8, 2>(p, st);
    case 11: return launch<1, 4, 4>(p, st);
    case 12: return launch<1, 2, 4>(p, st);
    case 13: return launch<1, 1, 4>(p, st);
    case 14: return launch<1, 1, 8>(p, st);
    case 15: return launch<1, 4, 2>(p, st);
    case 16: return launch<1, 2, 8>(p, st);
    case 17: return launch<1, 16, 2>(p, st);
    case 20: return launch<16, 2, 4>(p, st);
    case 21: return launch<16, 1, 4>(p, st);
    case 22: return launch<16, 4, 2>(p, st);
    case 23: return launch<16, 1, 8>(p, st);
    case 30: return launch<8, 2, 4>(p, st);
    case 31: return launch<8, 4, 2>(p, st);
    case 32: return launch<8, 1, 4>(p, st);
    case 33: return launch<8, 8, 2>(p, st);
    default: return BGNN_E_RANGE;
  }
}
#endif
```

### bridged_gnn_amd/ktgnn.py

```python
import math
import os
import weakref

import torch
import torch.nn.functional as F
from torch import nn

from . import ops

__all__ = ["Linear", "AdaptedConv", "KTGNN_no_complement"]


def _plist(module):
    pl = module.__dict__.get("_bgnn_plist")
    if pl is None:
        pl = list(module.parameters())
        module.__dict__["_bgnn_plist"] = pl
    return pl


def _forget_plists(root):
    for m in root.modules():
        m.__dict__.pop("_bgnn_plist", None)

# ... 540 lines not shown
        if colsum is not None and (fuse is None and epilogue is not None or self.root_weight or self.normalize):
            raise ValueError("colsum needs the fused epilogue path")
        res = self.aggregate(h_t2s, h_s2t, csr, mask_u8, want_alpha=return_alpha, epilogue=fuse, colsum=colsum)
        out, alpha = res if return_alpha else (res, None)
        out = out[:, : self.out_channels]
        if self.root_weight and x_r is not None:
            out = out + self.lin_r(x_r.float())
        if self.normalize:
            out = F.normalize(out, p=2.0, dim=-1)
        if epilogue is not None and fuse is None:
            sc, sh, relu = epilogue
            out = out * sc + sh
            out = F.relu(out) if relu else out
        return (out, alpha) if return_alpha else out

    def __repr__(self):
        return f"{self.__class__.__name__}({self.in_channels}, {self.out_channels})"


class KTGNN_no_complement(_PlistHooks, nn.Module):

    def __init__(self, num_features, num_classes=2, layer_num=2, hidden=64, root_weight=False, dim_share=300,
                 step=1, hidden_o=128, hidden_u=128, use_dist_loss=False, cached_edges=True, dropout=0.5,
                 use_bn=False, need_complement=False):
        super().__init__()
        if need_complement:
            raise NotImplementedError("Adapted_complementor is out of scope (never enabled by the reference drivers)")
        self.cached_edges, self.dropout, self.use_bn, self.need_complement = cached_edges, dropout, use_bn, False
        self.convs = nn.ModuleList()
        self.bns = nn.ModuleList()
        dim_in = dim_share
        if layer_num == 1:
            self.convs.append(AdaptedConv(dim_in, num_classes, root_weight=root_weight))
        else:
            for num in range(layer_num - 1):
                self.convs.append(AdaptedConv(dim_in if num == 0 else hidden, hidden, root_weight=root_weight))
                if self.use_bn:
                    self.bns.append(nn.BatchNorm1d(hidden))
        self.clf_base = AdaptedConv(hidden, num_classes, root_weight=root_weight)
        self.clf_target = AdaptedConv(hidden, num_classes, root_weight=root_weight)
        self.clf_transformer = nn.Sequential(
            Linear(hidden, hidden, bias=True), nn.BatchNorm1d(hidden), nn.ReLU(), Linear(hidden, hidden, bias=True))
        self.edge_index1 = self.edge_index2 = self.edge_index = None
        self._csr = None
        self._arena = None
        self._stage = classifier_stage.ClassifierStage(self)

    def reset_parameters(self):
        for conv in self.convs:
            conv.reset_parameters()
        for bn in self.bns:
            bn.reset_parameters()
        self.clf_base.reset_parameters()
        self.clf_target.reset_parameters()
        for l in self.clf_transformer:
            if isinstance(l, (Linear, nn.BatchNorm1d)):
                l.reset_parameters()

    def graph_partition(self, edge_index, central_mask, add_self_loop=True):
        if not edge_index.is_cuda:
            raise RuntimeError("graph_partition runs on CUDA(HIP) tensors only; there is no CPU path")
        if add_self_loop:
            n = central_mask.shape[0]
            edge_index = edge_index[:, edge_index[0] != edge_index[1]]
            loop = torch.arange(n, dtype=torch.int64, device=edge_index.device)
            edge_index = torch.cat([edge_index, torch.stack([loop, loop])], dim=1)
        m1 = central_mask[edge_index[1]]
        e1, e2 = edge_index[:, m1], edge_index[:, ~m1]
        return e1, e2, torch.cat((e1, e2), dim=-1)

    def _prepare(self, data):
        if self.cached_edges and self._csr is not None:
            return self._csr
        csr = ops.build_dst_csr(data.edge_index, data.central_mask.shape[0], rewrite_self_loops=True)
        if self.cached_edges:
            self._csr = csr
        return csr

    def _hidden(self, x, csr, central_mask, want_sums=False, arena=None):
        sums = None
        for ind, conv in enumerate(self.convs):
            sums_in, sums = sums, None
            if self.use_bn and not self.training and not (torch.is_grad_enabled() and any(p.requires_grad for p in _plist(conv))):
                sc, sh = bn_eval_affine(self.bns[ind])
                if arena is None:
                    arena = ops.ZeroArena(x.device, (len(self.convs) + 3) * (2 * ops.pad4(max(x.shape[1], conv.out_channels)) + 2))
                if sums_in is None and x.dtype == torch.float32 and x.stride(1) == 1 and x.shape[1] % 4 == 0:
                    sums_in = self._input_domain_sums(x, central_mask, arena)
                if not (conv.root_weight or conv.normalize):
                    sums = arena.take(2 * ops.pad4(conv.out_channels) + 2)
                x = conv(x, None, central_mask=central_mask, csr=csr, epilogue=(sc, sh, True), colsum=sums, sums=sums_in)
            else:
                if (ind == 0 and sums_in is None and torch.is_grad_enabled() and not x.requires_grad and x.dtype == torch.float32
                        and x.stride(1) == 1 and x.shape[1] % 4 == 0):
                    sums_in = self._input_domain_sums(x, central_mask, ops.ZeroArena(x.device, 2 * x.shape[1] + 2) if self._input_sums_miss(x, central_mask) else None)
                x = conv(x, None, central_mask=central_mask, csr=csr, sums=sums_in)
                if self.use_bn and self.training and torch.is_grad_enabled():
                    x = bn_relu_dropout_train(x, self.bns[ind], True, self.dropout)
                else:
                    if self.use_bn:
                        x = self.bns[ind](x)
                    x = F.relu(x)
                    x = F.dropout(x, p=self.dropout, training=self.training)
        self._arena = arena
        return (x, sums) if want_sums else x

    def _input_sums_miss(self, x, central_mask):
        if torch.cuda.is_current_stream_capturing() or not getattr(self, "cache_input_sums", True):
            return True
        c = getattr(self, "_xsum_cache", None)
        return not (c is not None and c[0]() is x and c[1] == x._version and c[2]() is central_mask and c[3] == central_mask._version)

    def _input_domain_sums(self, x, central_mask, arena):
        if torch.cuda.is_current_stream_capturing() or not getattr(self, "cache_input_sums", True):
            return ops.domain_sums(x, _as_u8(central_mask).contiguous(), out=arena.take(2 * x.shape[1] + 2))
        c = getattr(self, "_xsum_cache", None)
        if (c is not None and c[0]() is x and c[1] == x._version and c[2]() is central_mask and c[3] == central_mask._version):
            return c[4]
        sums = ops.domain_sums(x, _as_u8(central_mask).contiguous(), out=arena.take(2 * x.shape[1] + 2)).clone()
        self._xsum_cache = (weakref.ref(x), x._version, weakref.ref(central_mask), central_mask._version, sums)
        return sums

    def _transformer_to_target_tables(self, x, mask_u8, out, arena=None, sums_out=None):
        return self._stage.target_tables(x, mask_u8, out, arena, sums_out)

    def _composed_target_pack(self, din_pad):
        return self._stage.composed_target_pack(din_pad)

    def forward(self, data):
        x, central_mask = data.x, data.central_mask
        csr = self._prepare(data)
        x, sums_h = self._hidden(x, csr, central_mask, want_sums=True)
        x = x.contiguous()
        mask_u8 = _as_u8(central_mask).contiguous()
        stage = self._stage
        train = self.training and torch.is_grad_enabled()
        walk = stage.train_walk(opt_in=True) if (train and stage.plain and x.dtype == torch.float32) else None
        if walk is not None:
            sums_x = ops.domain_sums(_pad_cols4(x.detach()), mask_u8)
            tabs = stage.train_tables(x, mask_u8, sums_x, bn_relu_dropout_train)
            return (*stage.train_aggregate(walk, csr, mask_u8, tabs), None)
        if not stage.plain or torch.is_grad_enabled() or self.training:
            logits_base = self.clf_base(x, None, central_mask=central_mask, csr=csr)
            logits_target = self.clf_target(x, None, central_mask=central_mask, csr=csr)
            needs_grad = torch.is_grad_enabled() and (x.requires_grad or any(p.requires_grad for p in _plist(self.clf_transformer)))
            if train:
                l0, bn, _, l3 = self.clf_transformer
                xt = l3(bn_relu_dropout_train(l0(x), bn, True, 0.0))
            else:
                xt = self.clf_transformer(x) if (self.training or needs_grad) else stage.transformer_eval(x)
            logits_hat = self.clf_target(xt.contiguous(), None, central_mask=central_mask, csr=csr)
            return (F.log_softmax(logits_base, dim=1), F.log_softmax(logits_target, dim=1),
                    F.log_softmax(logits_hat, dim=1), None)
        t2s = torch.empty(x.shape[0], 3 * stage.ld, dtype=torch.float32, device=x.device)
        s2t = torch.empty_like(t2s)
        stage.eval_tables(x, mask_u8, sums_h, stage.views(t2s, s2t), self._arena)
        a_t2s, a_s2t = stage.attention()
        out3 = ops.adaptedconv_aggregate(t2s, s2t, a_t2s, a_s2t, csr, mask_u8, stage.C, stage.slope, heads=3,
                                         log_softmax=stage.fused_log_softmax)
        return (*stage.finish(out3), None)

    def graphed(self, data, warmup=2):
        if self.training:
            raise RuntimeError("graphed() captures the eval forward; call model.eval() first")
        with torch.no_grad():
            for _ in range(max(int(warmup), 1)):
                self.forward(data)
            torch.cuda.synchronize()
            g = torch.cuda.CUDAGraph()
            with torch.cuda.graph(g):
                out = self.forward(data)

        def replay():
            g.replay()
            return out
        replay.graph = g
        return replay

    def _drop_param_caches(self):
        for c in list(self.convs) + [self.clf_base, self.clf_target]:
            c._pack_key = None
        self._stage.drop_caches()
        for bn in list(self.bns) + [self.clf_transformer[1]]:
            bn._bgnn_affine = None
        _forget_plists(self)

    def invalidate_input_cache(self):
        self._xsum_cache = None

    def graphed_train_step(self, data, loss_fn, optimizer, warmup=3):
        if not self.training:
            raise RuntimeError("graphed_train_step() captures a training step; call model.train() first")
        if any(not g["capturable"] for g in optimizer.param_groups if "capturable" in g):
            raise RuntimeError("graphed_train_step() needs a capturable optimizer, e.g. torch.optim.Adam(params, capturable=True)")
        dev = data.x.device
        step = torch.zeros(1, dtype=torch.int64, device=dev)
        side = torch.cuda.Stream(device=dev)
        side.wait_stream(torch.cuda.current_stream(dev))
        _DROPOUT_STEP[0] = step
        try:
            with torch.cuda.stream(side):
                for _ in range(max(int(warmup), 1)):
                    step.add_(1)
                    optimizer.zero_grad(set_to_none=True)
                    loss_fn(self(data)).backward()
                    optimizer.step()
            torch.cuda.current_stream(dev).wait_stream(side)
            torch.cuda.synchronize(dev)
            g = torch.cuda.CUDAGraph()
            optimizer.zero_grad(set_to_none=True)
            with torch.cuda.graph(g):
                step.add_(1)
                loss = loss_fn(self(data))
                loss.backward()
                optimizer.step()
        finally:
            _DROPOUT_STEP[0] = None
        self._drop_param_caches()

        def replay():
            g.replay()
            self._drop_param_caches()
            return loss
        replay.graph, replay.step = g, step
        return replay

    def get_emb(self, data):
        return self._hidden(data.x, self._prepare(data), data.central_mask)


from . import classifier_stage
```

### bridged_gnn_amd/ops.py

```python
import os

import torch

from . import _lib as L

__all__ = ["DstCSR", "build_dst_csr", "domain_delta", "pack_transform_heads", "adaptedconv_transform", "adaptedconv_aggregate", "linear", "linear_supported", "linear_narrow_supported", "linear_narrow_transform", "narrow_transform_finish", "gram", "gram_supported", "rowdot", "transform_bwd_prep", "topk_edges_coalesced",
           "l2_normalize_rows", "cosine_topk", "mlp_pair_topk", "topk_edges", "coalesce", "gather_rows", "pad4",
           "sage_mean_aggregate", "sage_mean_aggregate_bwd", "rows_segment_add", "gcn_aggregate", "gcn_aggregate_bwd", "wide_heads_supported",
           "adaptedconv_aggregate_heads_wide", "adaptedconv_aggregate_heads_wide_bwd", "pair_csr", "pair_mlp_stats", "pair_mlp_loss",
           "pair_mlp_segsum", "pair_mlp_eval", "pair_mlp_count", "PAIR_MLP_WIDTH", "pair_cos_loss", "pair_cos_segsum", "pair_cos_count",
           "PAIR_COS_WIDTH"]


def pad4(n):
    return (int(n) + 3) // 4 * 4


HUB_THRESHOLD = 128
HUB_SEGMENT = 64


class DstCSR:

    def __init__(self, rowptr, col, eperm, num_edges, num_nodes):
# ... 345 lines not shown
                                              L.ptr(seed_dev) if seed_dev is not None else None,
                                              L.ptr(gx), D, L.ptr(gsum), L.stream())
    L.check(rc, "bgnn_bn_relu_dropout_bwd_f32")
    return gx, gsum.view(-1, 2 * D).sum(0)


def _bn_rows_args(x, totals, n_total, gamma, beta, eps, relu, p_drop, seed, seed_dev, row_ids, row_base):
    D = x.shape[1]
    if totals.dtype != torch.float64 or totals.numel() != 2 * D:
        raise RuntimeError(f"totals must be {2 * D} doubles (sum x | sum x^2 over all ranks' rows)")
    if row_ids is not None and (row_ids.dtype != torch.int64 or row_ids.numel() != x.shape[0]):
        raise RuntimeError("row_ids must hold one int64 global row number per local row")
    return (L.ptr(totals), int(n_total), L.ptr(gamma) if gamma is not None else None, L.ptr(beta) if beta is not None else None,
            float(eps), int(bool(relu)), float(p_drop), int(seed) & 0xFFFFFFFFFFFFFFFF, L.ptr(seed_dev) if seed_dev is not None else None,
            L.ptr(row_ids) if row_ids is not None else None, int(row_base))


def bn_colstats(x):
    N, D = x.shape
    acc = torch.empty(L.lib().bgnn_bn_acc_doubles(D), dtype=torch.float64, device=x.device)
    L.check(L.lib().bgnn_bn_colstats_f32(L.ptr_rows(x), N, D, x.stride(0), L.ptr(acc), L.stream()), "bgnn_bn_colstats_f32")
    return acc.view(-1, 2 * D).sum(0)


def bn_apply_rows(x, totals, n_total, gamma, beta, eps, relu, p_drop, seed, row_ids=None, row_base=0, momentum=0.0, running_mean=None,
                  running_var=None, seed_dev=None):
    N, D = x.shape
    y = torch.empty(N, D, dtype=torch.float32, device=x.device)
    a = _bn_rows_args(x, totals, n_total, gamma, beta, eps, relu, p_drop, seed, seed_dev, row_ids, row_base)
    rc = L.lib().bgnn_bn_apply_rows_f32(L.ptr_rows(x), N, D, x.stride(0), *a, float(momentum),
                                        L.ptr(running_mean) if running_mean is not None else None,
                                        L.ptr(running_var) if running_var is not None else None, L.ptr(y), D, L.stream())
    L.check(rc, "bgnn_bn_apply_rows_f32")
    return y


def bn_bwd_reduce_rows(x, grad_y, totals, n_total, gamma, beta, eps, relu, p_drop, seed, row_ids=None, row_base=0, seed_dev=None):
    N, D = x.shape
    gacc = torch.empty(L.lib().bgnn_bn_acc_doubles(D), dtype=torch.float64, device=x.device)
    a = _bn_rows_args(x, totals, n_total, gamma, beta, eps, relu, p_drop, seed, seed_dev, row_ids, row_base)
    rc = L.lib().bgnn_bn_bwd_reduce_rows_f32(L.ptr_rows(x), L.ptr_rows(grad_y), N, D, x.stride(0), grad_y.stride(0), *a, L.ptr(gacc), L.stream())
    L.check(rc, "bgnn_bn_bwd_reduce_rows_f32")
    return gacc.view(-1, 2 * D).sum(0)


def bn_bwd_apply_rows(x, grad_y, totals, gtotals, n_total, gamma, beta, eps, relu, p_drop, seed, row_ids=None, row_base=0, seed_dev=None):
    N, D = x.shape
    if gtotals.dtype != torch.float64 or gtotals.numel() != 2 * D:
        raise RuntimeError(f"gtotals must be {2 * D} doubles (sum g' | sum g'.xhat over all ranks' rows)")
    gx = torch.empty(N, D, dtype=torch.float32, device=x.device)
    a = _bn_rows_args(x, totals, n_total, gamma, beta, eps, relu, p_drop, seed, seed_dev, row_ids, row_base)
    rc = L.lib().bgnn_bn_bwd_apply_rows_f32(L.ptr_rows(x), L.ptr_rows(grad_y), N, D, x.stride(0), grad_y.stride(0), a[0], L.ptr(gtotals), *a[1:],
                                            L.ptr(gx), D, L.stream())
    L.check(rc, "bgnn_bn_bwd_apply_rows_f32")
    return gx


def rowdot(X, V):
    N, d = X.shape
    nv = V.shape[0]
    out = torch.empty(N, nv, dtype=torch.float32, device=X.device)
    rc = L.lib().bgnn_rowdot_f32(L.ptr_rows(X), X.stride(0), N, d, L.ptr(V), V.stride(0), nv, L.ptr(out), L.stream())
    L.check(rc, "bgnn_rowdot_f32")
    return out


def pack_transform_heads(heads, din_pad):
    D = heads[0]["W_s"].shape[0]
    din = heads[0]["W_s"].shape[1]
    ldh = pad4(D)
    dev = heads[0]["W_s"].device
    H = len(heads)
    Wp = torch.zeros(H * 2 * ldh, din_pad, dtype=torch.float32, device=dev)
    bp = torch.zeros(H * 2 * ldh, dtype=torch.float32, device=dev)
    gates = torch.zeros(H, 2, 2 * din_pad, dtype=torch.float32, device=dev)
    gconst = torch.zeros(H, 2, dtype=torch.float32, device=dev)
    for h, hd in enumerate(heads):
        if hd.get("gate_const") is not None:
            gconst[h, 0], gconst[h, 1] = hd["gate_const"]
        base = h * 2 * ldh
        Wp[base: base + D, :din] = hd["W_t"]
        Wp[base + ldh: base + ldh + D, :din] = hd["W_s"]
        if hd.get("b_t") is not None:
            bp[base: base + D] = hd["b_t"]
        if hd.get("b_s") is not None:
            bp[base + ldh: base + ldh + D] = hd["b_s"]
        for t, key in enumerate(("g_s2t", "g_t2s")):
            g = hd[key].reshape(-1)
            gates[h, t, :din] = g[:din]
            gates[h, t, din_pad: din_pad + din] = g[din:]
    return Wp, bp, gates, D, ldh, gconst


def adaptedconv_transform(x, mask_u8, delta, packed, out=None, sums=None, tail_single=(0, 0), tile_need=None):
    lib = L.lib()
    Wp, bp, gates, D, ldh, gconst = packed
    H = gates.shape[0]
    N, Din = x.shape
    dev = x.device
    if out is None:
        out = [(torch.empty(N, ldh, dtype=torch.float32, device=dev), torch.empty(N, ldh, dtype=torch.float32, device=dev))
               for _ in range(H)]
    row_stride = out[0][0].stride(0)
    for a, b in out:
        assert a.shape[0] >= N and b.shape[0] >= N and a.stride(0) == row_stride and b.stride(0) == row_stride
    small = torch.empty(H * (2 * ldh + 2) + 8, dtype=torch.float32, device=dev)
    o1 = out[1] if H > 1 else (None, None)
    if delta is None:
        if sums is None or sums.dtype != torch.float64 or sums.numel() != 2 * Din + 2:
            raise ValueError("adaptedconv_transform needs delta [Din] or the float64 domain sums [2*Din+2]")
        fn, first, name = lib.bgnn_adaptedconv_transform_sums_f32, sums, "bgnn_adaptedconv_transform_sums_f32"
    else:
        fn, first, name = lib.bgnn_adaptedconv_transform_f32, delta, "bgnn_adaptedconv_transform_f32"
    tail = (int(tail_single[0]), int(tail_single[1])) if delta is None else ()
    if delta is not None and tuple(tail_single) != (0, 0):
        raise ValueError("tail_single needs the sums form of the transform")
    if tile_need is not None:
        if delta is not None or tuple(tail_single) != (0, 0):
            raise ValueError("tile_need needs the sums form of the transform and no tail_single")
        if tile_need.dtype != torch.int32 or tile_need.numel() != (N + 31) // 32:
            raise ValueError("tile_need: one int32 per 32-row tile")
        fn, name, tail = lib.bgnn_adaptedconv_transform_need_f32, "bgnn_adaptedconv_transform_need_f32", (L.ptr(tile_need),)
    rc = fn(L.ptr(x), N, Din, x.stride(0), L.ptr(mask_u8), L.ptr(first), H, D, L.ptr(Wp), L.ptr(bp), L.ptr(gates), L.ptr(gconst),
            L.ptr_rows(out[0][1]), L.ptr_rows(out[0][0]), L.ptr_rows(o1[1]), L.ptr_rows(o1[0]), ldh, row_stride, *tail,
            L.ptr(small), L.stream())
    L.check(rc, name)
    return out


_P2_STATIC = os.environ.get("BGNN_P2_STATIC", "1") != "0"


def _tile_queue(dev):
    return torch.empty(8, dtype=torch.int32, device=dev)


def heads_log_softmax_supported(heads, D):
    return heads in (2, 3) and D <= 4


def _hub_shape_ok(D, ldh, ldo, heads, slope):
    if heads in (2, 3) and D <= 4 and ldh == 4 and ldo == 4:
        return True
    return heads == 1 and D > 32 and 0.0 <= slope <= 1.0


def adaptedconv_aggregate(h_t2s, h_s2t, a_t2s, a_s2t, csr, mask_u8, D, negative_slope=0.1, n_dst=None,
                          want_alpha=False, ep_scale=None, ep_shift=None, ep_relu=False, out=None,
                          row_begin=0, row_end=None, state_ms=None, part=0, heads=1, colsum=None, log_softmax=False,
                          park_begin=None):
    lib = L.lib()
    n_dst = csr.num_nodes if n_dst is None else int(n_dst)
    row_end = n_dst if row_end is None else int(row_end)
    ldh = h_t2s.stride(0) // heads
    ldo = pad4(D)
    dev = h_t2s.device
    if out is None:
        out = torch.empty(n_dst, heads * ldo, dtype=torch.float32, device=dev)
    assert h_t2s.stride(0) == h_s2t.stride(0) and h_t2s.stride(0) % heads == 0 and out.stride(0) % heads == 0
    alpha = torch.empty(csr.num_edges, dtype=torch.float32, device=dev) if want_alpha else None
    tq = _tile_queue(dev) if heads == 1 else None
    if row_end <= int(row_begin):
        return (out, alpha) if want_alpha else out
    if ((not want_alpha or heads == 1) and part in (0, 3) and int(row_begin) == 0 and row_end == csr.num_nodes == n_dst and h_t2s.shape[0] == n_dst
            and (ep_scale is None or heads == 1) and _hub_shape_ok(D, ldh, out.stride(0) // heads, heads, negative_slope)
            and os.environ.get("BGNN_HUB_ROWS", "1") != "0"):
        hubs = csr.hub_tables()
        if hubs is not None:
            hub_rows, seg_ptr, seg_bounds, seg_node = hubs
            nseg = int(seg_node.numel())
            wsb = lib.bgnn_aggregate_hub_workspace_bytes(nseg, heads, out.stride(0) // heads)
            ws = torch.empty(wsb, dtype=torch.uint8, device=dev)
            rc = lib.bgnn_adaptedconv_aggregate_hub_f32(
                L.ptr_rows(h_t2s), L.ptr_rows(h_s2t), ldh, L.ptr(a_t2s), L.ptr(a_s2t), L.ptr(csr.rowptr), L.ptr(csr.col),
                L.ptr(mask_u8), n_dst, D, float(negative_slope), L.ptr_rows(out), out.stride(0) // heads,
                L.ptr(ep_scale), L.ptr(ep_shift), 2 if log_softmax else (1 if ep_relu else 0),
                L.ptr(state_ms) if part == 3 else None, int(heads), L.ptr(colsum),
                L.ptr(tq), HUB_THRESHOLD, L.ptr(hub_rows), int(hub_rows.numel()),
                L.ptr(seg_ptr), L.ptr(seg_bounds), L.ptr(seg_node), nseg, L.ptr(alpha), L.ptr(ws), wsb, L.stream())
            L.check(rc, "bgnn_adaptedconv_aggregate_hub_f32")
            return (out, alpha) if want_alpha else out
    rc = lib.bgnn_adaptedconv_aggregate_bounded_f32(
        L.ptr_rows(h_t2s), L.ptr_rows(h_s2t), ldh, L.ptr(a_t2s), L.ptr(a_s2t), L.ptr(csr.rowptr), L.ptr(csr.col),
        L.ptr(mask_u8), int(row_begin), row_end, D, float(negative_slope), L.ptr_rows(out), out.stride(0) // heads, L.ptr(alpha),
        L.ptr(ep_scale), L.ptr(ep_shift), 2 if log_softmax else (1 if ep_relu else 0), L.ptr(state_ms), int(part),
        int(row_begin) if park_begin is None else int(park_begin), int(heads), L.ptr(colsum),
        L.ptr(tq) if not (part == 2 and _P2_STATIC) else None, min(int(h_t2s.shape[0]), int(h_s2t.shape[0])),
        csr.gather_hint() if (heads == 1 and D > 32 and part == 0) else 0, L.stream())
    L.check(rc, "bgnn_adaptedconv_aggregate_bounded_f32")
    return (out, alpha) if want_alpha else out


def adaptedconv_aggregate_bwd(h_t2s, h_s2t, a_t2s, a_s2t, csr, mask_u8, D, out, alpha, grad_out, negative_slope=0.1):
    lib = L.lib()
    dev = h_t2s.device
    da_t2s = torch.zeros(D, dtype=torch.float32, device=dev)
    da_s2t = torch.zeros(D, dtype=torch.float32, device=dev)
    grad_out = grad_out.contiguous()
    if D <= 128 and grad_out.stride(0) % 4 == 0 and grad_out.data_ptr() % 16 == 0 and h_t2s.shape[0] == csr.num_nodes:
        t_rowptr, t_eid, t_dst = csr.transposed()
        dh_t2s, dh_s2t = torch.empty_like(h_t2s), torch.empty_like(h_s2t)
        narrow = D <= 4 and h_t2s.stride(0) == 4 and out.stride(0) == 4 and grad_out.stride(0) == 4
        dh_, sh_ = (csr.hub_tables(), csr.transposed_hub_tables()) if (not narrow and os.environ.get("BGNN_HUB_ROWS", "1") != "0") else (None, None)
        if dh_ is not None or sh_ is not None:
            none4 = (None, None, None, None)
            d_rows, d_ptr, d_bounds, d_node = dh_ if dh_ is not None else none4
            s_rows, s_ptr, s_bounds, s_node = sh_ if sh_ is not None else none4
            nd = 0 if dh_ is None else int(d_node.numel())
            ns = 0 if sh_ is None else int(s_node.numel())
            wsb = lib.bgnn_aggregate_bwd_pull_hub_workspace_bytes(csr.num_nodes, csr.num_edges, h_t2s.stride(0), nd, ns)
            ws = torch.empty(wsb, dtype=torch.uint8, device=dev)
            rc = lib.bgnn_adaptedconv_aggregate_bwd_pull_hub_f32(
                L.ptr(h_t2s), L.ptr(h_s2t), h_t2s.stride(0), L.ptr(a_t2s), L.ptr(a_s2t), L.ptr(csr.rowptr), L.ptr(csr.col),
                L.ptr(mask_u8), L.ptr(t_rowptr), L.ptr(t_eid), L.ptr(t_dst), csr.num_nodes, csr.num_edges, D, float(negative_slope),
                L.ptr(out), out.stride(0), L.ptr(alpha), L.ptr(grad_out), grad_out.stride(0),
                L.ptr(dh_t2s), L.ptr(dh_s2t), L.ptr(da_t2s), L.ptr(da_s2t), HUB_THRESHOLD,
                L.ptr(d_rows), 0 if dh_ is None else int(d_rows.numel()), L.ptr(d_ptr), L.ptr(d_bounds), L.ptr(d_node), nd,
                L.ptr(s_rows), 0 if sh_ is None else int(s_rows.numel()), L.ptr(s_ptr), L.ptr(s_bounds), L.ptr(s_node), ns,
                L.ptr(ws), wsb, L.stream())
            L.check(rc, "bgnn_adaptedconv_aggregate_bwd_pull_hub_f32")
            return dh_t2s, dh_s2t, da_t2s, da_s2t
        wsb = lib.bgnn_aggregate_bwd_pull_workspace_bytes(csr.num_nodes, csr.num_edges, h_t2s.stride(0))
        ws = torch.empty(wsb, dtype=torch.uint8, device=dev)
        rc = lib.bgnn_adaptedconv_aggregate_bwd_pull_f32(
            L.ptr(h_t2s), L.ptr(h_s2t), h_t2s.stride(0), L.ptr(a_t2s), L.ptr(a_s2t), L.ptr(csr.rowptr), L.ptr(csr.col),
            L.ptr(mask_u8), L.ptr(t_rowptr), L.ptr(t_eid), L.ptr(t_dst), csr.num_nodes, csr.num_edges, D, float(negative_slope),
            L.ptr(out), out.stride(0), L.ptr(alpha), L.ptr(grad_out), grad_out.stride(0),
            L.ptr(dh_t2s), L.ptr(dh_s2t), L.ptr(da_t2s), L.ptr(da_s2t), L.ptr(ws), wsb, L.stream())
        L.check(rc, "bgnn_adaptedconv_aggregate_bwd_pull_f32")
        return dh_t2s, dh_s2t, da_t2s, da_s2t
    dh_t2s, dh_s2t = torch.zeros_like(h_t2s), torch.zeros_like(h_s2t)
    rc = lib.bgnn_adaptedconv_aggregate_bwd_f32(
        L.ptr(h_t2s), L.ptr(h_s2t), h_t2s.stride(0), L.ptr(a_t2s), L.ptr(a_s2t), L.ptr(csr.rowptr), L.ptr(csr.col),
        L.ptr(mask_u8), 0, csr.num_nodes, D, float(negative_slope), L.ptr(out), out.stride(0), L.ptr(alpha),
        L.ptr(grad_out), grad_out.stride(0), L.ptr(dh_t2s), L.ptr(dh_s2t), L.ptr(da_t2s), L.ptr(da_s2t), L.stream())
    L.check(rc, "bgnn_adaptedconv_aggregate_bwd_f32")
    return dh_t2s, dh_s2t, da_t2s, da_s2t


def adaptedconv_aggregate_heads_bwd(t2s, s2t, a_t2s, a_s2t, csr, mask_u8, D, heads, out, state_ms, grad_out, log_softmax,
                                    negative_slope=0.1):
    lib = L.lib()
    dev = t2s.device
    N = csr.num_nodes
    assert t2s.shape == (N, heads * 4) and t2s.is_contiguous() and s2t.is_contiguous() and out.is_contiguous() and grad_out.is_contiguous()
    da_t2s = torch.zeros(heads, D, dtype=torch.float32, device=dev)
    da_s2t = torch.zeros(heads, D, dtype=torch.float32, device=dev)
    dh_t2s, dh_s2t = torch.empty_like(t2s), torch.empty_like(s2t)
    t_rowptr, t_eid, t_dst = csr.transposed()
    dh_, sh_ = (csr.hub_tables(), csr.transposed_hub_tables()) if os.environ.get("BGNN_HUB_ROWS", "1") != "0" else (None, None)
    if dh_ is not None or sh_ is not None:
        none4 = (None, None, None, None)
        d_rows, d_ptr, d_bounds, d_node = dh_ if dh_ is not None else none4
        s_rows, s_ptr, s_bounds, s_node = sh_ if sh_ is not None else none4
        nd = 0 if dh_ is None else int(d_node.numel())
        ns = 0 if sh_ is None else int(s_node.numel())
        wsb = lib.bgnn_aggregate_heads_bwd_hub_workspace_bytes(N, csr.num_edges, heads, nd, ns)
        ws = torch.empty(wsb, dtype=torch.uint8, device=dev)
        rc = lib.bgnn_adaptedconv_aggregate_heads_bwd_hub_f32(
            L.ptr(t2s), L.ptr(s2t), L.ptr(a_t2s), L.ptr(a_s2t), L.ptr(csr.rowptr), L.ptr(csr.col), L.ptr(mask_u8),
            L.ptr(t_rowptr), L.ptr(t_dst), N, csr.num_edges, D, heads, float(negative_slope),
            L.ptr(out), L.ptr(state_ms), L.ptr(grad_out), int(bool(log_softmax)), L.ptr(dh_t2s), L.ptr(dh_s2t),
            L.ptr(da_t2s), L.ptr(da_s2t), HUB_THRESHOLD,
            L.ptr(d_rows), 0 if dh_ is None else int(d_rows.numel()), L.ptr(d_ptr), L.ptr(d_bounds), L.ptr(d_node), nd,
            L.ptr(s_rows), 0 if sh_ is None else int(s_rows.numel()), L.ptr(s_ptr), L.ptr(s_bounds), L.ptr(s_node), ns,
            L.ptr(ws), wsb, L.stream())
        L.check(rc, "bgnn_adaptedconv_aggregate_heads_bwd_hub_f32")
        return dh_t2s, dh_s2t, da_t2s, da_s2t
    wsb = lib.bgnn_aggregate_heads_bwd_workspace_bytes(N, csr.num_edges, heads)
    ws = torch.empty(wsb, dtype=torch.uint8, device=dev)
    rc = lib.bgnn_adaptedconv_aggregate_heads_bwd_f32(
        L.ptr(t2s), L.ptr(s2t), L.ptr(a_t2s), L.ptr(a_s2t), L.ptr(csr.rowptr), L.ptr(csr.col), L.ptr(mask_u8),
        L.ptr(t_rowptr), L.ptr(t_eid), L.ptr(t_dst), N, csr.num_edges, D, heads, float(negative_slope),
        L.ptr(out), L.ptr(state_ms), L.ptr(grad_out), int(bool(log_softmax)), L.ptr(dh_t2s), L.ptr(dh_s2t),
        L.ptr(da_t2s), L.ptr(da_s2t), L.ptr(ws), wsb, L.stream())
    L.check(rc, "bgnn_adaptedconv_aggregate_heads_bwd_f32")
    return dh_t2s, dh_s2t, da_t2s, da_s2t


def wide_heads_supported(heads, D):
    return heads in (2, 3) and 4 < int(D) <= 32


def adaptedconv_aggregate_heads_wide(t2s, s2t, a_t2s, a_s2t, csr, mask_u8, D, heads, negative_slope=0.1):
    lib = L.lib()
    N, ld = csr.num_nodes, pad4(D)
    assert t2s.shape == (N, heads * ld) and s2t.shape == t2s.shape and t2s.is_contiguous() and s2t.is_contiguous()
    out = torch.empty(N, heads * ld, dtype=torch.float32, device=t2s.device)
    ms = torch.empty(N, heads, 2, dtype=torch.float32, device=t2s.device)
    rc = lib.bgnn_adaptedconv_aggregate_heads_wide_f32(
        L.ptr(t2s), L.ptr(s2t), ld, L.ptr(a_t2s), L.ptr(a_s2t), L.ptr(csr.rowptr), L.ptr(csr.col), L.ptr(mask_u8),
        N, int(D), int(heads), float(negative_slope), L.ptr(out), L.ptr(ms), L.stream())
    L.check(rc, "bgnn_adaptedconv_aggregate_heads_wide_f32")
    return out, ms


def adaptedconv_aggregate_heads_wide_bwd(t2s, s2t, a_t2s, a_s2t, csr, mask_u8, D, heads, out, state_ms, grad_out,
                                         negative_slope=0.1):
    lib = L.lib()
    dev = t2s.device
    N, ld = csr.num_nodes, pad4(D)
    assert t2s.shape == (N, heads * ld) and t2s.is_contiguous() and s2t.is_contiguous() and out.is_contiguous() and grad_out.is_contiguous()
    da_t2s = torch.empty(heads, D, dtype=torch.float32, device=dev)
    da_s2t = torch.empty(heads, D, dtype=torch.float32, device=dev)
    dh_t2s, dh_s2t = torch.empty_like(t2s), torch.empty_like(s2t)
    t_rowptr, _, t_dst = csr.transposed()
    wsb = lib.bgnn_aggregate_heads_wide_bwd_workspace_bytes(N, heads, ld)
    ws = torch.empty(wsb, dtype=torch.uint8, device=dev)
    rc = lib.bgnn_adaptedconv_aggregate_heads_wide_bwd_f32(
        L.ptr(t2s), L.ptr(s2t), ld, L.ptr(a_t2s), L.ptr(a_s2t), L.ptr(csr.rowptr), L.ptr(csr.col), L.ptr(mask_u8),
        L.ptr(t_rowptr), L.ptr(t_dst), N, int(D), int(heads), float(negative_slope), L.ptr(out), L.ptr(state_ms), L.ptr(grad_out),
        L.ptr(dh_t2s), L.ptr(dh_s2t), L.ptr(da_t2s), L.ptr(da_s2t), L.ptr(ws), wsb, L.stream())
    L.check(rc, "bgnn_adaptedconv_aggregate_heads_wide_bwd_f32")
    return dh_t2s, dh_s2t, da_t2s, da_s2t


def l2_normalize_rows(q, eps=1e-8):
    out = torch.empty_like(q)
    rc = L.lib().bgnn_l2_normalize_rows_f32(L.ptr(q), q.shape[0], q.shape[1], float(eps), L.ptr(out), L.stream())
    L.check(rc, "bgnn_l2_normalize_rows_f32")
    return out


_COS_D = (32, 64, 128, 256)


def _pad_cols(t, d):
    if t.shape[1] == d:
        return t.contiguous()
    out = torch.zeros(t.shape[0], d, dtype=t.dtype, device=t.device)
    out[:, : t.shape[1]] = t
    return out


def cosine_topk(qn_query, qn_cand, k, apply_sigmoid=True):
    lib = L.lib()
    d = qn_query.shape[1]
    dk = next((c for c in _COS_D if c >= d), None)
    if dk is None:
        raise ValueError("embedding width > 256 unsupported")
    qq, qc = _pad_cols(qn_query, dk), _pad_cols(qn_cand, dk)
    Nq, Nc = qq.shape[0], qc.shape[0]
# ... 541 lines not shown
```

### include/bgnn.h

```cpp
#ifndef BGNN_H_
#define BGNN_H_
#include <stddef.h>
#include <stdint.h>

#ifdef __cplusplus
extern "C" {
#endif

#define BGNN_VERSION 113
#define BGNN_E_NULL (-1)
#define BGNN_E_SHAPE (-2)
#define BGNN_E_WORKSPACE (-3)
#define BGNN_E_ALIGN (-4)
#define BGNN_E_RANGE (-5)

int bgnn_version(void);
const char* bgnn_error_string(int code);
const char* bgnn_source_hash(void);

size_t bgnn_csr_workspace_bytes(int64_t N, int64_t E);
int bgnn_build_dst_csr(const int64_t* edge_index, int64_t E, int64_t N, int rewrite_self_loops,
                       int32_t* rowptr, int32_t* col, int32_t* eperm_opt, int64_t* E_out_dev,
                       void* ws, size_t ws_bytes, void* stream);

int bgnn_domain_sums_f64(const float* x, int64_t N, int32_t Din, int64_t ldx, const uint8_t* mask,
                         double* sums_io , void* stream);
size_t bgnn_domain_sums_workspace_bytes(int32_t Din);
int bgnn_domain_sums_ws_f64(const float* x, int64_t N, int32_t Din, int64_t ldx, const uint8_t* mask,
                            double* sums_io , void* ws, size_t ws_bytes, void* stream);
int bgnn_domain_delta_f32(const double* sums , int32_t Din, float* delta, void* stream);
int bgnn_linear_f32(const float* x, int64_t N, int32_t Din, int64_t ldx, const float* W, const float* bias,
                    int32_t Dout, int relu, const uint8_t* mask_opt, double* colsum_opt,
                    float* out, int64_t ldo, void* stream);
int bgnn_linear_narrow_transform_f32(const float* x, int64_t N, int32_t Din, int64_t ldx, const float* W,
                                     const float* bias, int32_t Dout, int relu, const uint8_t* mask,
                                     double* colsum, const float* Wp2, const float* gates2, float* raw, void* stream);
int bgnn_classifier_stage_f32(const float* x, int64_t N, int32_t Din, int64_t ldx, const uint8_t* mask,
                              const double* sums_x, int32_t sk_heads, int32_t sk_D, const float* sk_Wp,
                              const float* sk_bias, const float* sk_gates, const float* sk_gate_const_opt,
                              float* h_s2t_0, float* h_t2s_0, float* h_s2t_1, float* h_t2s_1, int64_t sk_ldh,
                              int64_t sk_row_stride, const float* W, const float* bias, int32_t Dout, int relu,
                              double* colsum, const float* Wp2, const float* gates2, float* raw, float* small_ws,
                              void* stream);
int bgnn_narrow_transform_finish_f32(const float* raw, int64_t N, const uint8_t* mask, const double* sums,
                                     int32_t Din, const float* Wp2, const float* bias2, const float* gates2,
                                     const float* gate_const_opt, float* h_s2t, float* h_t2s, int64_t row_stride,
                                     float* small_ws, void* stream);
size_t bgnn_gram_workspace_bytes(int32_t p, int32_t q);
int bgnn_gram_f32(const float* A, int64_t lda, int32_t p, const float* B, int64_t ldb, int32_t q, int64_t N,
                  float* out , void* ws, size_t ws_bytes, void* stream);
int64_t bgnn_bn_acc_doubles(int32_t D);
int bgnn_bn_relu_dropout_f32(const float* x, int64_t N, int32_t D, int64_t ldx, const float* gamma_opt,
                             const float* beta_opt, float eps, int relu, float p_drop, uint64_t seed, const uint64_t* seed_dev_opt,
                             float momentum, float* running_mean_opt, float* running_var_opt,
                             float* y, int64_t ldy, double* stats, void* stream);
int bgnn_bn_relu_dropout_bwd_f32(const float* x, const float* grad_y, int64_t N, int32_t D, int64_t ldx, int64_t ldg,
                                 const double* stats, const float* gamma_opt, const float* beta_opt, float eps,
                                 int relu, float p_drop, uint64_t seed, const uint64_t* seed_dev_opt, float* grad_x, int64_t ldgx,
                                 double* gsum, void* stream);
int bgnn_bn_colstats_f32(const float* x, int64_t n_rows, int32_t D, int64_t ldx, double* acc, void* stream);
int bgnn_bn_apply_rows_f32(const float* x, int64_t n_rows, int32_t D, int64_t ldx, const double* totals, int64_t n_total,
                           const float* gamma_opt, const float* beta_opt, float eps, int relu, float p_drop, uint64_t seed,
                           const uint64_t* seed_dev_opt, const int64_t* row_ids_opt, int64_t row_base,
                           float momentum, float* running_mean_opt, float* running_var_opt,
                           float* y, int64_t ldy, void* stream);
int bgnn_bn_bwd_reduce_rows_f32(const float* x, const float* grad_y, int64_t n_rows, int32_t D, int64_t ldx, int64_t ldg,
                                const double* totals, int64_t n_total, const float* gamma_opt, const float* beta_opt,
                                float eps, int relu, float p_drop, uint64_t seed, const uint64_t* seed_dev_opt,
                                const int64_t* row_ids_opt, int64_t row_base, double* gacc, void* stream);
int bgnn_bn_bwd_apply_rows_f32(const float* x, const float* grad_y, int64_t n_rows, int32_t D, int64_t ldx, int64_t ldg,
                               const double* totals, const double* gtotals, int64_t n_total, const float* gamma_opt,
                               const float* beta_opt, float eps, int relu, float p_drop, uint64_t seed,
                               const uint64_t* seed_dev_opt, const int64_t* row_ids_opt, int64_t row_base,
                               float* grad_x, int64_t ldgx, void* stream);
size_t bgnn_transform_bwd_prep_workspace_bytes(int64_t N, int32_t p);
int bgnn_transform_bwd_prep_f32(const float* x, int64_t ldx, int64_t N, int32_t din, const float* G_s2t, const float* G_t2s,
                                int64_t ldg, int32_t D, const uint8_t* mask, const float* gx ,
                                const float* gconst , const float* wd , const double* counts ,
                                float* Gall, int32_t p, int64_t ld_gall, float* side_opt, int64_t ld_side,
                                float* ex_opt , void* ws_opt, size_t ws_bytes, void* stream);
int bgnn_transform_bwd_consts_f32(const float* W_s, const float* W_t, const float* g1, const float* g2, const float* delta,
                                  int32_t D, int32_t din, float* gx, float* gconst, float* wd, void* stream);
int bgnn_transform_bwd_finish_f32(const float* dWall, const float* ex, const float* W_s, const float* W_t, const float* g1,
                                  const float* g2, const float* delta, int32_t D, int32_t din, int32_t p, float* dW_s,
                                  float* dW_t, float* dg1, float* dg2, float* db_s_opt, float* db_t_opt, float* wcat_t,
                                  int64_t ld_wcat, void* stream);
int bgnn_rowdot_f32(const float* X, int64_t ldx, int64_t N, int32_t d, const float* V, int64_t ldv, int32_t nv,
                    float* out , void* stream);
int bgnn_adaptedconv_transform_f32(const float* x, int64_t N, int32_t Din, int64_t ldx,
                                   const uint8_t* mask, const float* delta,
                                   int32_t n_heads, int32_t D, const float* Wp, const float* bias_p,
                                   const float* gates, const float* gate_const_opt,
                                   float* h_s2t_0, float* h_t2s_0, float* h_s2t_1, float* h_t2s_1,
                                   int64_t ldh, int64_t row_stride, float* small_ws, void* stream);
int bgnn_adaptedconv_transform_sums_f32(const float* x, int64_t N, int32_t Din, int64_t ldx,
                                        const uint8_t* mask, const double* sums,
                                        int32_t n_heads, int32_t D, const float* Wp, const float* bias_p,
                                        const float* gates, const float* gate_const_opt,
                                        float* h_s2t_0, float* h_t2s_0, float* h_s2t_1, float* h_t2s_1,
                                        int64_t ldh, int64_t row_stride, int64_t n_tail_t2s, int64_t n_tail_s2t,
                                        float* small_ws, void* stream);
int bgnn_adaptedconv_transform_need_f32(const float* x, int64_t N, int32_t Din, int64_t ldx,
                                        const uint8_t* mask, const double* sums,
                                        int32_t n_heads, int32_t D, const float* Wp, const float* bias_p,
                                        const float* gates, const float* gate_const_opt,
                                        float* h_s2t_0, float* h_t2s_0, float* h_s2t_1, float* h_t2s_1,
                                        int64_t ldh, int64_t row_stride, const int32_t* tile_need_opt,
                                        float* small_ws, void* stream);

int bgnn_adaptedconv_aggregate_f32(const float* h_t2s, const float* h_s2t, int64_t ldh,
                                   const float* a_t2s, const float* a_s2t,
                                   const int32_t* rowptr, const int32_t* col, const uint8_t* mask,
                                   int64_t row_begin, int64_t row_end, int32_t D, float negative_slope,
                                   float* out, int64_t ldo, float* alpha_opt,
                                   const float* ep_scale_opt, const float* ep_shift_opt, int ep_relu,
                                   float* state_ms_opt, int part, int64_t park_begin, int32_t heads, double* colsum_opt,
                                   uint32_t* tile_queue_opt, void* stream);

int bgnn_adaptedconv_aggregate_bounded_f32(const float* h_t2s, const float* h_s2t, int64_t ldh,
                                           const float* a_t2s, const float* a_s2t,
                                           const int32_t* rowptr, const int32_t* col, const uint8_t* mask,
                                           int64_t row_begin, int64_t row_end, int32_t D, float negative_slope,
                                           float* out, int64_t ldo, float* alpha_opt,
                                           const float* ep_scale_opt, const float* ep_shift_opt, int ep_relu,
                                           float* state_ms_opt, int part, int64_t park_begin, int32_t heads, double* colsum_opt,
                                           uint32_t* tile_queue_opt, int64_t table_rows, int32_t gather_hint, void* stream);

size_t bgnn_aggregate_hub_workspace_bytes(int64_t n_segments, int32_t heads, int64_t ldo);
int bgnn_adaptedconv_aggregate_hub_f32(const float* h_t2s, const float* h_s2t, int64_t ldh,
                                       const float* a_t2s, const float* a_s2t,
                                       const int32_t* rowptr, const int32_t* col, const uint8_t* mask,
                                       int64_t N, int32_t D, float negative_slope, float* out, int64_t ldo,
                                       const float* ep_scale_opt, const float* ep_shift_opt, int ep_relu,
                                       float* state_ms_opt, int32_t heads, double* colsum_opt,
                                       uint32_t* tile_queue_opt, int32_t hub_threshold, const int32_t* hub_rows,
                                       int64_t n_hubs, const int32_t* hub_seg_ptr, const int32_t* seg_bounds,
                                       const int32_t* seg_node, int64_t n_segments, float* alpha_opt,
                                       void* ws, size_t ws_bytes, void* stream);

int bgnn_adaptedconv_aggregate_bwd_f32(const float* h_t2s, const float* h_s2t, int64_t ldh,
                                       const float* a_t2s, const float* a_s2t,
                                       const int32_t* rowptr, const int32_t* col, const uint8_t* mask,
                                       int64_t row_begin, int64_t row_end, int32_t D, float negative_slope,
                                       const float* out, int64_t ldo, const float* alpha,
                                       const float* grad_out, int64_t ldg,
                                       float* dh_t2s, float* dh_s2t, float* da_t2s, float* da_s2t,
                                       void* stream);

size_t bgnn_aggregate_bwd_pull_workspace_bytes(int64_t N, int64_t E, int64_t ldh);
int bgnn_adaptedconv_aggregate_bwd_pull_f32(const float* h_t2s, const float* h_s2t, int64_t ldh,
                                            const float* a_t2s, const float* a_s2t,
                                            const int32_t* rowptr, const int32_t* col, const uint8_t* mask,
                                            const int32_t* t_rowptr, const int32_t* t_eid, const int32_t* t_dst,
                                            int64_t N, int64_t E, int32_t D, float negative_slope,
                                            const float* out, int64_t ldo, const float* alpha,
                                            const float* grad_out, int64_t ldg,
                                            float* dh_t2s, float* dh_s2t, float* da_t2s, float* da_s2t,
                                            void* ws, size_t ws_bytes, void* stream);

size_t bgnn_aggregate_bwd_pull_hub_workspace_bytes(int64_t N, int64_t E, int64_t ldh, int64_t d_segments, int64_t s_segments);
int bgnn_adaptedconv_aggregate_bwd_pull_hub_f32(const float* h_t2s, const float* h_s2t, int64_t ldh,
                                                const float* a_t2s, const float* a_s2t,
                                                const int32_t* rowptr, const int32_t* col, const uint8_t* mask,
                                                const int32_t* t_rowptr, const int32_t* t_eid, const int32_t* t_dst,
                                                int64_t N, int64_t E, int32_t D, float negative_slope,
                                                const float* out, int64_t ldo, const float* alpha,
                                                const float* grad_out, int64_t ldg,
                                                float* dh_t2s, float* dh_s2t, float* da_t2s, float* da_s2t,
                                                int32_t hub_threshold,
                                                const int32_t* d_hub_rows, int64_t d_n_hubs, const int32_t* d_hub_seg_ptr,
                                                const int32_t* d_seg_bounds, const int32_t* d_seg_node, int64_t d_n_segments,
                                                const int32_t* s_hub_rows, int64_t s_n_hubs, const int32_t* s_hub_seg_ptr,
                                                const int32_t* s_seg_bounds, const int32_t* s_seg_node, int64_t s_n_segments,
                                                void* ws, size_t ws_bytes, void* stream);

size_t bgnn_aggregate_heads_bwd_workspace_bytes(int64_t N, int64_t E, int32_t heads);
int bgnn_adaptedconv_aggregate_heads_bwd_f32(const float* h_t2s, const float* h_s2t, const float* a_t2s, const float* a_s2t,
                                             const int32_t* rowptr, const int32_t* col, const uint8_t* mask,
                                             const int32_t* t_rowptr, const int32_t* t_eid, const int32_t* t_dst,
                                             int64_t N, int64_t E, int32_t D, int32_t heads, float negative_slope,
                                             const float* out, const float* state_ms, const float* grad_out,
                                             int log_softmax, float* dh_t2s, float* dh_s2t, float* da_t2s,
                                             float* da_s2t, void* ws, size_t ws_bytes, void* stream);
size_t bgnn_aggregate_heads_bwd_hub_workspace_bytes(int64_t N, int64_t E, int32_t heads, int64_t d_segments, int64_t s_segments);
int bgnn_adaptedconv_aggregate_heads_bwd_hub_f32(const float* h_t2s, const float* h_s2t, const float* a_t2s, const float* a_s2t,
                                                 const int32_t* rowptr, const int32_t* col, const uint8_t* mask,
                                                 const int32_t* t_rowptr, const int32_t* t_dst,
                                                 int64_t N, int64_t E, int32_t D, int32_t heads, float negative_slope,
                                                 const float* out, const float* state_ms, const float* grad_out,
                                                 int log_softmax, float* dh_t2s, float* dh_s2t, float* da_t2s, float* da_s2t,
                                                 int32_t hub_threshold,
                                                 const int32_t* d_hub_rows, int64_t d_n_hubs, const int32_t* d_hub_seg_ptr,
                                                 const int32_t* d_seg_bounds, const int32_t* d_seg_node, int64_t d_n_segments,
                                                 const int32_t* s_hub_rows, int64_t s_n_hubs, const int32_t* s_hub_seg_ptr,
                                                 const int32_t* s_seg_bounds, const int32_t* s_seg_node, int64_t s_n_segments,
                                                 void* ws, size_t ws_bytes, void* stream);

int bgnn_adaptedconv_aggregate_heads_wide_f32(const float* h_t2s, const float* h_s2t, int64_t ldh,
                                              const float* a_t2s, const float* a_s2t,
                                              const int32_t* rowptr, const int32_t* col, const uint8_t* mask,
                                              int64_t N, int32_t D, int32_t heads, float negative_slope,
                                              float* out, float* state_ms, void* stream);
size_t bgnn_aggregate_heads_wide_bwd_workspace_bytes(int64_t N, int32_t heads, int64_t ldh);
int bgnn_adaptedconv_aggregate_heads_wide_bwd_f32(const float* h_t2s, const float* h_s2t, int64_t ldh,
                                                  const float* a_t2s, const float* a_s2t,
                                                  const int32_t* rowptr, const int32_t* col, const uint8_t* mask,
                                                  const int32_t* t_rowptr, const int32_t* t_dst,
                                                  int64_t N, int32_t D, int32_t heads, float negative_slope,
                                                  const float* out, const float* state_ms, const float* grad_out,
                                                  float* dh_t2s, float* dh_s2t, float* da_t2s, float* da_s2t,
                                                  void* ws, size_t ws_bytes, void* stream);

int bgnn_sage_mean_aggregate_f32(const float* tbl, int64_t ldt, int64_t n_tbl, const float* root_opt, int64_t ldr,
                                 const int32_t* rowptr, const int32_t* col, int64_t n_rows, int32_t D, int mean,
                                 int epilogue, float p_drop, uint64_t seed, const uint64_t* seed_dev_opt,
                                 float* out, int64_t ldo, void* stream);
size_t bgnn_sage_mean_aggregate_bwd_workspace_bytes(int64_t n_rows, int32_t D);
int bgnn_sage_mean_aggregate_bwd_f32(const float* y, int64_t ldy, const float* grad_y, int64_t ldgy,
                                     const int32_t* rowptr, int64_t n_rows, const int32_t* t_rowptr, const int32_t* t_col,
                                     int64_t n_src, int32_t D, int epilogue, float p_drop,
                                     float* grad_tbl, int64_t ldgt, float* grad_root, int64_t ldgr,
                                     void* ws, size_t ws_bytes, void* stream);
int bgnn_sage_mean_aggregate_rows_f32(const float* tbl, int64_t ldt, int64_t n_tbl, const float* root_opt, int64_t ldr,
                                      const int32_t* rowptr, const int32_t* col, int64_t n_rows, int32_t D, int mean,
                                      int epilogue, float p_drop, uint64_t seed, const uint64_t* seed_dev_opt,
                                      const int64_t* row_id_opt, float* out, int64_t ldo, void* stream);
int bgnn_rows_segment_add_f32(const float* src, int64_t lds, int64_t n_src, const int32_t* seg_ptr, const int32_t* idx,
                              const int32_t* row, int64_t n_seg, int32_t D, int accumulate, float* dst, int64_t ldd, int64_t n_dst,
                              void* stream);

size_t bgnn_gcn_aggregate_workspace_bytes(int64_t n_seg, int32_t D);
int bgnn_gcn_aggregate_f32(const float* tbl, int64_t ldt, int64_t n_tbl, const float* bias_opt, const int32_t* rowptr,
                           const int32_t* col, const float* dinv, int64_t n_dinv, int64_t n_rows, int32_t D,
                           int epilogue, float p_drop, uint64_t seed, const uint64_t* seed_dev_opt,
                           int32_t hub_threshold, const int32_t* hub_rows_opt, int64_t n_hubs,
                           const int32_t* hub_seg_ptr_opt, const int32_t* seg_bounds_opt, int64_t n_seg,
                           void* ws_opt, size_t ws_bytes, float* out, int64_t ldo, void* stream);
int bgnn_gcn_aggregate_bwd_f32(const float* y, int64_t ldy, const float* grad_y, int64_t ldgy, int64_t n_rows,
                               const int32_t* t_rowptr, const int32_t* t_col, const float* dinv, int64_t n_dinv,
                               int64_t n_src, int32_t D, int epilogue, float p_drop,
                               int32_t hub_threshold, const int32_t* hub_rows_opt, int64_t n_hubs,
                               const int32_t* hub_seg_ptr_opt, const int32_t* seg_bounds_opt, int64_t n_seg,
                               void* ws_opt, size_t ws_bytes, float* g, int64_t ldg, float* grad_tbl, int64_t ldgt,
                               void* stream);
int bgnn_gcn_aggregate_rows_f32(const float* tbl, int64_t ldt, int64_t n_tbl, const float* bias_opt, const int32_t* rowptr,
                                const int32_t* col, const float* dinv, int64_t n_dinv, int64_t n_rows, int32_t D,
                                int epilogue, float p_drop, uint64_t seed, const uint64_t* seed_dev_opt,
                                int32_t hub_threshold, const int32_t* hub_rows_opt, int64_t n_hubs,
                                const int32_t* hub_seg_ptr_opt, const int32_t* seg_bounds_opt, int64_t n_seg,
                                void* ws_opt, size_t ws_bytes, const int64_t* row_id_opt, float* out, int64_t ldo, void* stream);

int bgnn_l2_normalize_rows_f32(const float* q, int64_t n, int32_t d, float eps, float* out, void* stream);
size_t bgnn_topk_workspace_bytes(int64_t Nq, int64_t Nc, int32_t k);
int bgnn_cosine_topk_f32(const float* qn_query, const float* qn_cand, int64_t Nq, int64_t Nc,
                         int32_t d, int32_t k, int apply_sigmoid,
                         int64_t* idx_out , float* val_out ,
                         int32_t* n_fallback_opt, void* ws, size_t ws_bytes, void* stream);
int bgnn_mlp_pair_topk_f32(const float* A_cand , const float* B_query ,
                           const float* bn_scale, const float* bn_shift, const float* w2, float b2,
                           int64_t Nq, int64_t Nc, int32_t H, int32_t k, int apply_sigmoid,
                           int64_t* idx_out, float* val_out, int32_t* n_fallback_opt,
                           void* ws, size_t ws_bytes, void* stream);

int bgnn_topk_edges_i64(const int64_t* idx, int64_t Nq, int32_t k, int64_t cand_base, int64_t query_base,
                        int64_t* edge_index_out, void* stream);
size_t bgnn_topk_edges_coalesced_workspace_bytes(int64_t Nq, int32_t k);
int bgnn_topk_edges_coalesced_i64(const int64_t* idx, int64_t Nq, int32_t k, int64_t Nc, int64_t cand_base, int64_t query_base,
                                  int64_t* edge_index_out, void* ws, size_t ws_bytes, void* stream);

int bgnn_gather_rows_f32(const float* src, int64_t src_rows, int64_t ld_src, const int64_t* idx, int64_t n,
                         int32_t row_floats, float* dst, int64_t ld_dst, void* stream);

size_t bgnn_coalesce_workspace_bytes(int64_t E);
int bgnn_coalesce_i64(int64_t* edge_index, int64_t E, int64_t num_nodes, int64_t* E_out_dev,
                      void* ws, size_t ws_bytes, void* stream);

size_t bgnn_pair_mlp_workspace_bytes(int64_t P);
size_t bgnn_pair_mlp_count_workspace_bytes(int64_t m1, int64_t m2);
int bgnn_pair_mlp_stats_f32(const float* A, int64_t lda, int64_t nA, const float* B, int64_t ldb, int64_t nB, const int64_t* idx1,
                            const int64_t* idx2, int64_t P, float momentum, float* run_mean_opt, float* run_var_opt, double* stats,
                            void* ws, size_t ws_bytes, void* stream);
int bgnn_pair_mlp_loss_f32(const float* A, int64_t lda, int64_t nA, const float* B, int64_t ldb, int64_t nB, const int64_t* idx1,
                           const int64_t* idx2, const uint8_t* y, int64_t P, const double* stats, const float* g2, const float* be2,
                           const float* w2, const float* b2, float eps, float* p_out, float* dl_out, double* sums, void* ws,
                           size_t ws_bytes, void* stream);
int bgnn_pair_mlp_segsum_f32(const float* own, int64_t ld_own, int64_t n_own, const float* other, int64_t ld_other, int64_t n_other,
                             const int32_t* rowptr, const int32_t* perm, const int64_t* idx_other, int64_t P, const float* dl,
                             const double* stats, const double* sums, const float* g2, const float* be2, const float* w2, float eps,
                             float* S, int64_t ld_s, void* stream);
int bgnn_pair_mlp_eval_f32(const float* A, int64_t lda, int64_t nA, const float* B, int64_t ldb, int64_t nB, const int64_t* idx1,
                           const int64_t* idx2, const uint8_t* y_opt, int64_t P, const float* scale2, const float* shift2,
// ... 56 lines not shown
```

Baseline: 50.19 billion edges/s.

## Pad 3-head classifier tables to 64-byte rows and add buffer-load fast aggregate kernel

Allocates the eval-time t2s/s2t classifier tables with a 16-float row stride instead of 12, so each node's three heads fill one 64-byte aligned row. A new specialized 3-head aggregation kernel uses buffer-resource loads with shift-based row offsets, prefetches the next column indices with inline asm, and uses 32-bit tile indexing. A strided entry point carries row stride and edge count through to the existing kernels. The padding spends a third more memory per table, and the inline asm and waitcnt scheduling add fragility in exchange for fewer partial-cacheline gathers and cheaper address math.

Measured after the change: 49.94 billion edges/s. Within noise of the previous version (-0.5%).

```diff
diff --git a/bridged_gnn_amd/_lib.py b/bridged_gnn_amd/_lib.py
--- a/bridged_gnn_amd/_lib.py
+++ b/bridged_gnn_amd/_lib.py
@@ -48,7 +48,11 @@
                                                _P, _I64, _P, _P, _P, _INT, _P, _INT, _I64, _I32, _P, _P, _P]),
     "bgnn_adaptedconv_aggregate_bounded_f32": (_INT, [_P, _P, _I64, _P, _P, _P, _P, _P, _I64, _I64, _I32, _F32,
                                                        _P, _I64, _P, _P, _P, _INT, _P, _INT, _I64, _I32, _P, _P, _I64, _I32, _P]),
+    "bgnn_adaptedconv_aggregate_strided_f32": (_INT, [_P, _P, _I64, _P, _P, _P, _P, _P, _I64, _I64, _I32, _F32,
+                                                       _P, _I64, _P, _P, _P, _INT, _P, _INT, _I64, _I32, _P, _P, _I64, _I32, _I64, _I64, _P]),
     "bgnn_aggregate_hub_workspace_bytes": (C.c_size_t, [_I64, _I32, _I64]),
+    "bgnn_adaptedconv_aggregate_hub_strided_f32": (_INT, [_P, _P, _I64, _P, _P, _P, _P, _P, _I64, _I32, _F32, _P, _I64, _P, _P, _INT, _P, _I32, _P,
+                                                           _P, _I32, _P, _I64, _P, _P, _P, _I64, _P, _P, C.c_size_t, _I64, _P]),
     "bgnn_adaptedconv_aggregate_hub_f32": (_INT, [_P, _P, _I64, _P, _P, _P, _P, _P, _I64, _I32, _F32, _P, _I64, _P, _P, _INT, _P, _I32, _P,
                                                    _P, _I32, _P, _I64, _P, _P, _P, _I64, _P, _P, C.c_size_t, _P]),
     "bgnn_adaptedconv_aggregate_bwd_f32": (_INT, [_P, _P, _I64, _P, _P, _P, _P, _P, _I64, _I64, _I32, _F32,
diff --git a/bridged_gnn_amd/classifier_stage.py b/bridged_gnn_amd/classifier_stage.py
--- a/bridged_gnn_amd/classifier_stage.py
+++ b/bridged_gnn_amd/classifier_stage.py
@@ -23,6 +23,12 @@
     def views(self, t2s, s2t):
         ld = self.ld
         return [(t2s[:, j * ld:(j + 1) * ld], s2t[:, j * ld:(j + 1) * ld]) for j in range(3)]
+
+    def alloc_eval_tables(self, rows, device):
+        w = 3 * self.ld
+        stride = 16 if (w == 12 and os.environ.get("BGNN_HEADS_ROW64", "1") != "0") else w
+        both = torch.empty(2, rows, stride, dtype=torch.float32, device=device)
+        return both[0, :, :w], both[1, :, :w]
 
     def attention(self, autograd=False):
         if autograd:
diff --git a/bridged_gnn_amd/csrc/bgnn_aggregate.hip b/bridged_gnn_amd/csrc/bgnn_aggregate.hip
--- a/bridged_gnn_amd/csrc/bgnn_aggregate.hip
+++ b/bridged_gnn_amd/csrc/bgnn_aggregate.hip
@@ -40,6 +40,8 @@
   uint32_t tbl_bytes, off_t2s, off_s2t;
   int32_t gather_hint;
   uint32_t dead_off;
+  int64_t row_stride;
+  int64_t num_edges;
 };
 
 __device__ __forceinline__ float leaky(float v, float slope) { return v > 0.f ? v : v * slope; }
@@ -752,7 +754,7 @@
   }
 }
 
-template <int HEADS, int EP, int U>
+template <int HEADS, int EP, int U, bool A16 = true>
 __global__ __launch_bounds__(256) void agg_heads_lanes_kernel(AggParams p) {
   constexpr int GL = EP * HEADS, GPW = 64 / GL, RPB = 4 * GPW;
   const int lane = threadIdx.x & 63, wave = threadIdx.x >> 6;
@@ -761,7 +763,11 @@
   const bool lane_on = g < GPW;
   const int64_t ntiles = (p.row_end - p.row_begin + p.n_vrows + RPB - 1) / RPB;
   bgnn::XcdRange tr = bgnn::xcd_pos_range(ntiles);
-  const int64_t rs = (int64_t)HEADS * p.ldh;
+  const int64_t rs = p.row_stride > 0 ? p.row_stride : (int64_t)HEADS * p.ldh;
+  auto row4 = [](const float* q) {
+    if constexpr (A16) return *reinterpret_cast<const float4*>(q);
+    else return make_float4(q[0], q[1], q[2], q[3]);
+  };
   for (int64_t pos = tr.begin; pos < tr.end; pos += tr.step) {
     const int64_t tile = bgnn::xcd_tile_of(pos, ntiles);
     if (tile < 0) continue;
@@ -787,7 +793,7 @@
     a4.y = p.D > 1 ? av[h * p.D + 1] : 0.f;
     a4.z = p.D > 2 ? av[h * p.D + 2] : 0.f;
     a4.w = p.D > 3 ? av[h * p.D + 3] : 0.f;
-    const float4 hi = *reinterpret_cast<const float4*>(H + node * rs + h * p.ldh);
+    const float4 hi = row4(H + node * rs + h * p.ldh);
     float4 acc = make_float4(0.f, 0.f, 0.f, 0.f);
     float m = -INFINITY, s = 0.f;
     if (p.mode == 2 && rvalid && !virt && sub == 0) {
@@ -806,7 +812,7 @@
       }
 #pragma unroll
       for (int u = 0; u < U; ++u)
-        v[u] = id[u] >= 0 ? *reinterpret_cast<const float4*>(H + (int64_t)id[u] * rs + h * p.ldh) : make_float4(0.f, 0.f, 0.f, 0.f);
+        v[u] = id[u] >= 0 ? row4(H + (int64_t)id[u] * rs + h * p.ldh) : make_float4(0.f, 0.f, 0.f, 0.f);
       float lg_[U], cm = -INFINITY;
 #pragma unroll
       for (int u = 0; u < U; ++u) {
@@ -878,6 +884,142 @@
   }
 }
 
+template <int HEADS, bool S64>
+__global__ __launch_bounds__(256) void agg_heads_fast_kernel(AggParams p) {
+  constexpr int EP = 2, U = 4, GL = EP * HEADS, GPW = 64 / GL, RPB = 4 * GPW;
+  const int lane = threadIdx.x & 63, wave = threadIdx.x >> 6;
+  const int g = lane / GL, lg = lane % GL;
+  const int sub = lg / HEADS, h = lg % HEADS;
+  const bool lane_on = g < GPW;
+  const int32_t row0 = (int32_t)p.row_begin, row1 = (int32_t)p.row_end;
+  const int32_t ntiles = (row1 - row0 + RPB - 1) / RPB;
+  const int32_t xcd = blockIdx.x % 8, slot = blockIdx.x / 8, nslots = ((int32_t)gridDim.x + 7 - xcd) / 8;
+  const int32_t seg_len = ((ntiles + 7) / 8 + bgnn::XCD_NSEG - 1) / bgnn::XCD_NSEG;
+  const uint32_t stride = S64 ? 64u : (uint32_t)p.row_stride * 4u;
+  const __amdgpu_buffer_rsrc_t rt = __builtin_amdgcn_make_buffer_rsrc(const_cast<char*>(p.tbl_base), (short)0, (int)p.tbl_bytes, 0x00020000);
+  auto row_off = [&](uint32_t id) { return S64 ? id << 6 : id * stride; };
+  const float slope = p.slope;
+  float4 aS, aT;
+  aS.x = p.a_t2s[h * p.D]; aT.x = p.a_s2t[h * p.D];
+  aS.y = p.D > 1 ? p.a_t2s[h * p.D + 1] : 0.f; aT.y = p.D > 1 ? p.a_s2t[h * p.D + 1] : 0.f;
+  aS.z = p.D > 2 ? p.a_t2s[h * p.D + 2] : 0.f; aT.z = p.D > 2 ? p.a_s2t[h * p.D + 2] : 0.f;
+  aS.w = p.D > 3 ? p.a_t2s[h * p.D + 3] : 0.f; aT.w = p.D > 3 ? p.a_s2t[h * p.D + 3] : 0.f;
+  for (int32_t j = slot; j < bgnn::XCD_NSEG * seg_len; j += nslots) {
+    const int32_t sg = j / seg_len, tile = (sg * 8 + xcd) * seg_len + (j - sg * seg_len);
+    if (tile >= ntiles) continue;
+    const int32_t i = row0 + tile * RPB + wave * GPW + g;
+    const bool rvalid = lane_on && i < row1;
+    const int32_t ic = rvalid ? i : row0;
+    const bool dom_s = p.mask[ic] != 0;
+    const int32_t beg = rvalid ? p.rowptr[ic] : 0;
+    const int32_t end = rvalid ? p.rowptr[ic + 1] : 0;
+    const float4 a4 = dom_s ? aS : aT;
+    const uint32_t lbase = (dom_s ? p.off_t2s : p.off_s2t) + (uint32_t)h * 16u;
+    const float4 hi4 = __builtin_bit_cast(float4, __builtin_amdgcn_raw_buffer_load_b128(rt, lbase + row_off((uint32_t)ic), 0, 0));
+    float hx = hi4.x, hy = hi4.y, hz = hi4.z, hw = hi4.w;
+    float ax = 0.f, ay = 0.f, az = 0.f, aw = 0.f;
+    float m = -INFINITY, s = 0.f;
+    const int32_t niter = (end - beg + EP * U - 1) / (EP * U);
+    int32_t nw = 0;
+#pragma unroll
+    for (int q = 0; q < GPW; ++q) nw = max(nw, __builtin_amdgcn_readlane(niter, q * GL));
+    auto load_id = [&](int32_t ee) {
+      uint32_t id;
+      const uint32_t eoff = (uint32_t)max(min(ee, end - 1), 0) * 4u;
+      asm volatile("global_load_dword %0, %1, %2" : "=v"(id) : "v"(eoff), "s"(p.col) : "memory");
+      return id;
+    };
+    int32_t e = beg + sub;
+    uint32_t id[U];
+#pragma unroll
+    for (int u = 0; u < U; ++u) id[u] = 0u;
+    if (nw > 0) {
+#pragma unroll
+      for (int u = 0; u < U; ++u) id[u] = (uint32_t)p.col[max(min(e + u * EP, end - 1), 0)];
+    }
+    for (int32_t it = 0; it < nw; ++it) {
+      bool ok[U];
+      float4 v[U];
+#pragma unroll
+      for (int u = 0; u < U; ++u) {
+        ok[u] = e + u * EP < end;
+        const uint32_t off = ok[u] ? lbase + row_off(id[u]) : p.dead_off;
+        v[u] = __builtin_bit_cast(float4, __builtin_amdgcn_raw_buffer_load_b128(rt, off, 0, 0));
+      }
+      asm volatile("" : "+v"(hx), "+v"(hy), "+v"(hz), "+v"(hw) : : "memory");
+      __builtin_amdgcn_sched_barrier(0);
+      e += EP * U;
+      uint32_t nid[U];
+#pragma unroll
+      for (int u = 0; u < U; ++u) nid[u] = load_id(e + u * EP);
+      __builtin_amdgcn_sched_barrier(0);
+      float lg_[U], cm = -INFINITY;
+#pragma unroll
+      for (int u = 0; u < U; ++u) {
+        float t = a4.x * leaky(v[u].x + hx, slope);
+        t = fmaf(a4.y, leaky(v[u].y + hy, slope), t);
+        t = fmaf(a4.z, leaky(v[u].z + hz, slope), t);
+        t = fmaf(a4.w, leaky(v[u].w + hw, slope), t);
+        lg_[u] = ok[u] ? t : -INFINITY;
+        cm = fmaxf(cm, lg_[u]);
+      }
+      const float mn = fmaxf(m, cm);
+      const float sc = (m == mn) ? 1.f : __expf(m - mn);
+      s *= sc;
+      ax *= sc; ay *= sc; az *= sc; aw *= sc;
+#pragma unroll
+      for (int u = 0; u < U; ++u) {
+        const float pe = (lg_[u] == -INFINITY) ? 0.f : __expf(lg_[u] - mn);
+        s += pe;
+        ax = fmaf(pe, v[u].x, ax); ay = fmaf(pe, v[u].y, ay);
+        az = fmaf(pe, v[u].z, az); aw = fmaf(pe, v[u].w, aw);
+      }
+      m = mn;
+      __builtin_amdgcn_sched_barrier(0);
+      asm volatile("s_waitcnt vmcnt(0)"
+                   : "+v"(nid[0]), "+v"(nid[1]), "+v"(nid[2]), "+v"(nid[3]), "+v"(m), "+v"(s), "+v"(ax), "+v"(ay), "+v"(az), "+v"(aw)
+                   : : "memory");
+#pragma unroll
+      for (int u = 0; u < U; ++u) id[u] = nid[u];
+    }
+    float4 acc = make_float4(ax, ay, az, aw);
+#pragma unroll
+    for (int off = 1; off < EP; off <<= 1) {
+      const int src = (sub ^ off) * HEADS + h + g * GL;
+      const int from = lane_on ? src : lane;
+      const float m2 = __shfl(m, from), s2 = __shfl(s, from);
+      float4 b;
+      b.x = __shfl(acc.x, from); b.y = __shfl(acc.y, from); b.z = __shfl(acc.z, from); b.w = __shfl(acc.w, from);
+      const float mn = fmaxf(m, m2);
+      const float c1 = (m == mn) ? 1.f : __expf(m - mn), c2 = (m2 == mn) ? 1.f : __expf(m2 - mn);
+      s = s * c1 + s2 * c2;
+      acc.x = acc.x * c1 + b.x * c2; acc.y = acc.y * c1 + b.y * c2;
+      acc.z = acc.z * c1 + b.z * c2; acc.w = acc.w * c1 + b.w * c2;
+      m = mn;
+    }
+    if (rvalid && sub == 0) {
+      const float inv = 1.f / (s + 1e-16f);
+      float4 r = make_float4(acc.x * inv, acc.y * inv, acc.z * inv, acc.w * inv);
+      if (p.ep_relu == 2) {
+        float mx = r.x;
+        if (p.D > 1) mx = fmaxf(mx, r.y);
+        if (p.D > 2) mx = fmaxf(mx, r.z);
+        if (p.D > 3) mx = fmaxf(mx, r.w);
+        float se = expf(r.x - mx);
+        if (p.D > 1) se += expf(r.y - mx);
+        if (p.D > 2) se += expf(r.z - mx);
+        if (p.D > 3) se += expf(r.w - mx);
+        const float lse = logf(se);
+        r.x = r.x - mx - lse;
+        r.y = p.D > 1 ? r.y - mx - lse : 0.f;
+        r.z = p.D > 2 ? r.z - mx - lse : 0.f;
+        r.w = p.D > 3 ? r.w - mx - lse : 0.f;
+      }
+      *reinterpret_cast<float4*>(p.out + ((uint32_t)i * (uint32_t)HEADS + (uint32_t)h) * 4u) = r;
+    }
+  }
+}
+
 inline int tq_chunk_for(int64_t ntiles, int64_t grid) {
   static const int forced = [] { const char* e = getenv("BGNN_AGG_CHUNK"); return e ? atoi(e) : 0; }();
   (void)ntiles; (void)grid;
@@ -898,7 +1040,8 @@
   const int64_t ntiles = (p.row_end - p.row_begin + p.n_vrows + RPB - 1) / RPB;
   int64_t grid = ntiles < cap ? (ntiles + 7) / 8 * 8 : cap;
   if (grid < 8) grid = 8;
-  hipLaunchKernelGGL((agg_heads_lanes_kernel<HEADS, EP, U>), dim3((unsigned)grid), dim3(256), 0, st, p);
+  if (p.row_stride & 3) hipLaunchKernelGGL((agg_heads_lanes_kernel<HEADS, EP, U, false>), dim3((unsigned)grid), dim3(256), 0, st, p);
+  else hipLaunchKernelGGL((agg_heads_lanes_kernel<HEADS, EP, U>), dim3((unsigned)grid), dim3(256), 0, st, p);
   BGNN_LAUNCH_CHECK();
   return 0;
 }
@@ -969,6 +1112,7 @@
   const char* lo = a < b ? a : b;
   const int64_t span = (int64_t)((a < b ? b : a) - lo) + table_rows * p.ldh * 4;
   if (span > lim32 || p.row_end * p.ldo * 4 > lim32) return false;
+  if (p.num_edges * 4 > lim32) return false;
   p.tbl_base = lo;
   p.tbl_bytes = (uint32_t)span;
   p.off_t2s = (uint32_t)(a - lo);
@@ -976,6 +1120,66 @@
   const int64_t lane_max = (span - table_rows * p.ldh * 4) + p.ldh * 4, dead = (((int64_t)1 << 32) - 16) - lane_max;
   p.dead_off = dead >= span ? (uint32_t)dead : 0u;
   return true;
+}
+
+static bool heads_fast_plan_on() {
+  static const bool on = [] { const char* e = getenv("BGNN_AGG_FAST"); return !(e && atoi(e) == 0); }();
+  return on;
+}
+static bool heads_fast_plan(AggParams& p, int64_t table_rows) {
+  if (table_rows <= 0 || p.num_edges <= 0) return false;
+  if (p.mode != 0 || p.n_vrows != 0 || p.hub_threshold != 0 || p.alpha != nullptr || p.state_ms != nullptr) return false;
+  if (p.row_begin < 0 || p.row_end > table_rows) return false;
+  const int64_t stride = (p.row_stride > 0 ? p.row_stride : (int64_t)p.heads * p.ldh) * 4;
+  if ((stride & 15) || stride < (int64_t)p.heads * 16) return false;
+  const int64_t lim32 = ((int64_t)1 << 32) - 1, dead = lim32 + 1 - 65536;
+  if (table_rows > lim32 / stride || p.num_edges > lim32 / 4 || p.row_end > lim32 / ((int64_t)p.heads * 16)) return false;
+  const char* a = reinterpret_cast<const char*>(p.h_t2s);
+  const char* b = reinterpret_cast<const char*>(p.h_s2t);
+  const char* lo = a < b ? a : b;
+  const char* hi = a < b ? b : a;
+  if ((int64_t)(hi - lo) > dead) return false;
+  const int64_t span = (int64_t)(hi - lo) + table_rows * stride;
+  if (span > dead) return false;
+  p.tbl_base = lo;
+  p.tbl_bytes = (uint32_t)span;
+  p.off_t2s = (uint32_t)(a - lo);
+  p.off_s2t = (uint32_t)(b - lo);
+  p.dead_off = (uint32_t)dead;
+  return true;
+}
+
+template <int HEADS>
+int launch_heads_fast(const AggParams& p, hipStream_t st) {
+  constexpr int RPB = 4 * (64 / (2 * HEADS));
+  const bool s64 = (p.row_stride > 0 ? p.row_stride : (int64_t)HEADS * p.ldh) == 16;
+  static const int per_cu_max = [] {
+    int a = 0, b = 0;
+    if (hipOccupancyMaxActiveBlocksPerMultiprocessor(&a, agg_heads_fast_kernel<HEADS, true>, 256, 0) != hipSuccess || a < 1) return 0;
+    if (hipOccupancyMaxActiveBlocksPerMultiprocessor(&b, agg_heads_fast_kernel<HEADS, false>, 256, 0) != hipSuccess || b < 1) return 0;
+    int per_cu = a < b ? a : b;
+    if (per_cu > 8) per_cu = 8;
+    return per_cu;
+  }();
+  static const int n_cu = [] {
+    int dev = 0;
+    hipDeviceProp_t prop;
+    if (hipGetDevice(&dev) != hipSuccess || hipGetDeviceProperties(&prop, dev) != hipSuccess) return 0;
+    return prop.multiProcessorCount;
+  }();
+  static const int forced = [] { const char* e = getenv("BGNN_HEADS_BLOCKS_PER_CU"); return e ? atoi(e) : 0; }();
+  static const int scattered = [] { const char* e = getenv("BGNN_HEADS_BLOCKS_SCATTERED"); return e ? atoi(e) : 0; }();
+  int per_cu = per_cu_max;
+  if (forced > 0 && forced < per_cu) per_cu = forced;
+  else if (p.gather_hint == 2 && scattered > 0 && scattered < per_cu) per_cu = scattered;
+  const int64_t cap = (per_cu_max > 0 && n_cu > 0) ? (int64_t)per_cu * n_cu / 8 * 8 : 2048;
+  const int64_t ntiles = (p.row_end - p.row_begin + RPB - 1) / RPB;
+  int64_t grid = ntiles < cap ? (ntiles + 7) / 8 * 8 : cap;
+  if (grid < 8) grid = 8;
+  if (s64) hipLaunchKernelGGL((agg_heads_fast_kernel<HEADS, true>), dim3((unsigned)grid), dim3(256), 0, st, p);
+  else hipLaunchKernelGGL((agg_heads_fast_kernel<HEADS, false>), dim3((unsigned)grid), dim3(256), 0, st, p);
+  BGNN_LAUNCH_CHECK();
+  return 0;
 }
 
 template <int LF, bool ALPHA>
@@ -1147,7 +1351,11 @@
 
 static int dispatch_aggregate(const AggParams& p, hipStream_t st, int64_t table_rows = 0) {
   const int32_t D = p.D, heads = p.heads;
-  if (heads == 3 && D <= 4 && p.ldh == 4 && p.ldo == 4) return launch_heads<3, 2, 4>(p, st);
+  if (heads == 3 && D <= 4 && p.ldh == 4 && p.ldo == 4) {
+    AggParams q = p;
+    if (heads_fast_plan_on() && heads_fast_plan(q, table_rows)) return launch_heads_fast<3>(q, st);
+    return launch_heads<3, 2, 4>(p, st);
+  }
   if (heads == 2 && D <= 4 && p.ldh == 4 && p.ldo == 4) return launch_heads<2, 2, 4>(p, st);
   const int nv = (D + 3) / 4;
   if (nv <= 1) return launch<1, 4, 4>(p, st);
@@ -1191,8 +1399,11 @@
                           float* out, int64_t ldo, float* alpha_opt,
                           const float* ep_scale_opt, const float* ep_shift_opt, int ep_relu,
                           float* state_ms_opt, int part, int64_t park_begin, int32_t heads,
-                          double* colsum_opt, uint32_t* tile_queue_opt, int64_t table_rows, int32_t gather_hint, void* stream) {
+                          double* colsum_opt, uint32_t* tile_queue_opt, int64_t table_rows, int32_t gather_hint, void* stream,
+                          int64_t num_edges = 0, int64_t row_stride = 0) {
   if (colsum_opt && heads != 1) return BGNN_E_SHAPE;
+  if (num_edges < 0 || row_stride < 0) return BGNN_E_SHAPE;
+  if (row_stride > 0 && (!((heads == 3 || heads == 2) && D <= 4 && ldh == 4 && ldo == 4) || row_stride < (int64_t)heads * ldh)) return BGNN_E_SHAPE;
   if (part == 1 && (park_begin < row_begin || park_begin > row_end)) return BGNN_E_SHAPE;
   if (part < 0 || part > 3 || (part != 0 && (!state_ms_opt || alpha_opt))) return BGNN_E_NULL;
   if (part == 3 && !((heads == 3 || heads == 2) && D <= 4 && ldh == 4 && ldo == 4)) return BGNN_E_SHAPE;
@@ -1209,6 +1420,8 @@
               out, ldo, alpha_opt, ep_scale_opt, ep_shift_opt, ep_relu, tile_queue_opt, colsum_opt, heads, state_ms_opt, part,
               park_begin, 4};
   p.gather_hint = gather_hint;
+  p.row_stride = row_stride;
+  p.num_edges = num_edges;
   hipStream_t st = (hipStream_t)stream;
   if (tile_queue_opt) {
     hipError_t e = bgnn_zero_async(tile_queue_opt, 8 * sizeof(uint32_t), st);
@@ -1243,21 +1456,37 @@
                         ep_scale_opt, ep_shift_opt, ep_relu, state_ms_opt, part, park_begin, heads, colsum_opt, tile_queue_opt, table_rows, gather_hint, stream);
 }
 
+extern "C" int bgnn_adaptedconv_aggregate_strided_f32(const float* h_t2s, const float* h_s2t, int64_t ldh,
+                                                      const float* a_t2s, const float* a_s2t,
+                                                      const int32_t* rowptr, const int32_t* col, const uint8_t* mask,
+                                                      int64_t row_begin, int64_t row_end, int32_t D, float negative_slope,
+                                                      float* out, int64_t ldo, float* alpha_opt,
+                                                      const float* ep_scale_opt, const float* ep_shift_opt, int ep_relu,
+                                                      float* state_ms_opt, int part, int64_t park_begin, int32_t heads,
+                                                      double* colsum_opt, uint32_t* tile_queue_opt, int64_t table_rows, int32_t gather_hint,
+                                                      int64_t num_edges, int64_t row_stride, void* stream) {
+  if ((table_rows != 0 && table_rows < row_end) || gather_hint < 0 || gather_hint > 2) return BGNN_E_SHAPE;
+  return aggregate_impl(h_t2s, h_s2t, ldh, a_t2s, a_s2t, rowptr, col, mask, row_begin, row_end, D, negative_slope, out, ldo, alpha_opt,
+                        ep_scale_opt, ep_shift_opt, ep_relu, state_ms_opt, part, park_begin, heads, colsum_opt, tile_queue_opt, table_rows, gather_hint, stream,
+                        num_edges, row_stride);
+}
+
 extern "C" size_t bgnn_aggregate_hub_workspace_bytes(int64_t n_segments, int32_t heads, int64_t ldo) {
   const size_t nv = (size_t)(n_segments > 0 ? n_segments : 0), h = (size_t)(heads > 0 ? heads : 1);
   return bgnn_align_up(sizeof(float) * nv * h * (size_t)(ldo > 0 ? ldo : 0), 256) + bgnn_align_up(sizeof(float) * 2 * nv * h, 256) + 256;
 }
 
-extern "C" int bgnn_adaptedconv_aggregate_hub_f32(const float* h_t2s, const float* h_s2t, int64_t ldh,
-                                                  const float* a_t2s, const float* a_s2t,
-                                                  const int32_t* rowptr, const int32_t* col, const uint8_t* mask,
-                                                  int64_t N, int32_t D, float negative_slope, float* out, int64_t ldo,
-                                                  const float* ep_scale_opt, const float* ep_shift_opt, int ep_relu,
-                                                  float* state_ms_opt, int32_t heads, double* colsum_opt,
-                                                  uint32_t* tile_queue_opt, int32_t hub_threshold, const int32_t* hub_rows,
-                                                  int64_t n_hubs, const int32_t* hub_seg_ptr, const int32_t* seg_bounds,
-                                                  const int32_t* seg_node, int64_t n_segments, float* alpha_opt,
-                                                  void* ws, size_t ws_bytes, void* stream) {
+static int aggregate_hub_impl(const float* h_t2s, const float* h_s2t, int64_t ldh,
+                              const float* a_t2s, const float* a_s2t,
+                              const int32_t* rowptr, const int32_t* col, const uint8_t* mask,
+                              int64_t N, int32_t D, float negative_slope, float* out, int64_t ldo,
+                              const float* ep_scale_opt, const float* ep_shift_opt, int ep_relu,
+                              float* state_ms_opt, int32_t heads, double* colsum_opt,
+                              uint32_t* tile_queue_opt, int32_t hub_threshold, const int32_t* hub_rows,
+                              int64_t n_hubs, const int32_t* hub_seg_ptr, const int32_t* seg_bounds,
+                              const int32_t* seg_node, int64_t n_segments, float* alpha_opt,
+                              void* ws, size_t ws_bytes, int64_t row_stride, void* stream) {
+  if (row_stride < 0 || (row_stride > 0 && (heads < 2 || row_stride < (int64_t)heads * ldh))) return BGNN_E_SHAPE;
   if (!h_t2s || !h_s2t || !a_t2s || !a_s2t || !rowptr || !col || !mask || !out) return BGNN_E_NULL;
   if (alpha_opt && heads != 1) return BGNN_E_SHAPE;
   if (n_hubs > 0 && (!hub_rows || !hub_seg_ptr || !seg_bounds || !seg_node || !ws)) return BGNN_E_NULL;
@@ -1277,6 +1506,7 @@
               out, ldo, alpha_opt, ep_scale_opt, ep_shift_opt, ep_relu, tile_queue_opt, colsum_opt, heads, state_ms_opt, part,
               0, 4};
   p.hub_threshold = n_hubs > 0 ? hub_threshold : 0;
+  p.row_stride = row_stride;
   if (tile_queue_opt) {
     hipError_t e = bgnn_zero_async(tile_queue_opt, 8 * sizeof(uint32_t), st);
     if (e != hipSuccess) return (int)e;
@@ -1301,6 +1531,36 @@
   }
   BGNN_LAUNCH_CHECK();
   return 0;
+}
+
+extern "C" int bgnn_adaptedconv_aggregate_hub_f32(const float* h_t2s, const float* h_s2t, int64_t ldh,
+                                                  const float* a_t2s, const float* a_s2t,
+                                                  const int32_t* rowptr, const int32_t* col, const uint8_t* mask,
+                                                  int64_t N, int32_t D, float negative_slope, float* out, int64_t ldo,
+                                                  const float* ep_scale_opt, const float* ep_shift_opt, int ep_relu,
+                                                  float* state_ms_opt, int32_t heads, double* colsum_opt,
+                                                  uint32_t* tile_queue_opt, int32_t hub_threshold, const int32_t* hub_rows,
+                                                  int64_t n_hubs, const int32_t* hub_seg_ptr, const int32_t* seg_bounds,
+                                                  const int32_t* seg_node, int64_t n_segments, float* alpha_opt,
+                                                  void* ws, size_t ws_bytes, void* stream) {
+  return aggregate_hub_impl(h_t2s, h_s2t, ldh, a_t2s, a_s2t, rowptr, col, mask, N, D, negative_slope, out, ldo, ep_scale_opt, ep_shift_opt,
+                            ep_relu, state_ms_opt, heads, colsum_opt, tile_queue_opt, hub_threshold, hub_rows, n_hubs, hub_seg_ptr,
+                            seg_bounds, seg_node, n_segments, alpha_opt, ws, ws_bytes, 0, stream);
+}
+
+extern "C" int bgnn_adaptedconv_aggregate_hub_strided_f32(const float* h_t2s, const float* h_s2t, int64_t ldh,
+                                                          const float* a_t2s, const float* a_s2t,
+                                                          const int32_t* rowptr, const int32_t* col, const uint8_t* mask,
+                                                          int64_t N, int32_t D, float negative_slope, float* out, int64_t ldo,
+                                                          const float* ep_scale_opt, const float* ep_shift_opt, int ep_relu,
+                                                          float* state_ms_opt, int32_t heads, double* colsum_opt,
+                                                          uint32_t* tile_queue_opt, int32_t hub_threshold, const int32_t* hub_rows,
+                                                          int64_t n_hubs, const int32_t* hub_seg_ptr, const int32_t* seg_bounds,
+                                                          const int32_t* seg_node, int64_t n_segments, float* alpha_opt,
+                                                          void* ws, size_t ws_bytes, int64_t row_stride, void* stream) {
+  return aggregate_hub_impl(h_t2s, h_s2t, ldh, a_t2s, a_s2t, rowptr, col, mask, N, D, negative_slope, out, ldo, ep_scale_opt, ep_shift_opt,
+                            ep_relu, state_ms_opt, heads, colsum_opt, tile_queue_opt, hub_threshold, hub_rows, n_hubs, hub_seg_ptr,
+                            seg_bounds, seg_node, n_segments, alpha_opt, ws, ws_bytes, row_stride, stream);
 }
 
 #ifdef BGNN_TUNING
diff --git a/bridged_gnn_amd/ktgnn.py b/bridged_gnn_amd/ktgnn.py
--- a/bridged_gnn_amd/ktgnn.py
+++ b/bridged_gnn_amd/ktgnn.py
@@ -716,8 +716,7 @@
             logits_hat = self.clf_target(xt.contiguous(), None, central_mask=central_mask, csr=csr)
             return (F.log_softmax(logits_base, dim=1), F.log_softmax(logits_target, dim=1),
                     F.log_softmax(logits_hat, dim=1), None)
-        t2s = torch.empty(x.shape[0], 3 * stage.ld, dtype=torch.float32, device=x.device)
-        s2t = torch.empty_like(t2s)
+        t2s, s2t = stage.alloc_eval_tables(x.shape[0], x.device)
         stage.eval_tables(x, mask_u8, sums_h, stage.views(t2s, s2t), self._arena)
         a_t2s, a_s2t = stage.attention()
         out3 = ops.adaptedconv_aggregate(t2s, s2t, a_t2s, a_s2t, csr, mask_u8, stage.C, stage.slope, heads=3,
diff --git a/bridged_gnn_amd/ops.py b/bridged_gnn_amd/ops.py
--- a/bridged_gnn_amd/ops.py
+++ b/bridged_gnn_amd/ops.py
@@ -521,12 +521,17 @@
     lib = L.lib()
     n_dst = csr.num_nodes if n_dst is None else int(n_dst)
     row_end = n_dst if row_end is None else int(row_end)
-    ldh = h_t2s.stride(0) // heads
     ldo = pad4(D)
+    row_stride = 0
+    if heads_log_softmax_supported(heads, D) and h_t2s.stride(0) != heads * 4:
+        ldh, row_stride = 4, h_t2s.stride(0)
+    else:
+        ldh = h_t2s.stride(0) // heads
+        assert h_t2s.stride(0) % heads == 0
     dev = h_t2s.device
     if out is None:
         out = torch.empty(n_dst, heads * ldo, dtype=torch.float32, device=dev)
-    assert h_t2s.stride(0) == h_s2t.stride(0) and h_t2s.stride(0) % heads == 0 and out.stride(0) % heads == 0
+    assert h_t2s.stride(0) == h_s2t.stride(0) and out.stride(0) % heads == 0
     alpha = torch.empty(csr.num_edges, dtype=torch.float32, device=dev) if want_alpha else None
     tq = _tile_queue(dev) if heads == 1 else None
     if row_end <= int(row_begin):
@@ -540,23 +545,24 @@
             nseg = int(seg_node.numel())
             wsb = lib.bgnn_aggregate_hub_workspace_bytes(nseg, heads, out.stride(0) // heads)
             ws = torch.empty(wsb, dtype=torch.uint8, device=dev)
-            rc = lib.bgnn_adaptedconv_aggregate_hub_f32(
+            rc = lib.bgnn_adaptedconv_aggregate_hub_strided_f32(
                 L.ptr_rows(h_t2s), L.ptr_rows(h_s2t), ldh, L.ptr(a_t2s), L.ptr(a_s2t), L.ptr(csr.rowptr), L.ptr(csr.col),
                 L.ptr(mask_u8), n_dst, D, float(negative_slope), L.ptr_rows(out), out.stride(0) // heads,
                 L.ptr(ep_scale), L.ptr(ep_shift), 2 if log_softmax else (1 if ep_relu else 0),
                 L.ptr(state_ms) if part == 3 else None, int(heads), L.ptr(colsum),
                 L.ptr(tq), HUB_THRESHOLD, L.ptr(hub_rows), int(hub_rows.numel()),
-                L.ptr(seg_ptr), L.ptr(seg_bounds), L.ptr(seg_node), nseg, L.ptr(alpha), L.ptr(ws), wsb, L.stream())
-            L.check(rc, "bgnn_adaptedconv_aggregate_hub_f32")
+                L.ptr(seg_ptr), L.ptr(seg_bounds), L.ptr(seg_node), nseg, L.ptr(alpha), L.ptr(ws), wsb, int(row_stride), L.stream())
+            L.check(rc, "bgnn_adaptedconv_aggregate_hub_strided_f32")
             return (out, alpha) if want_alpha else out
-    rc = lib.bgnn_adaptedconv_aggregate_bounded_f32(
+    table_rows = int(h_t2s.shape[0]) if h_t2s.shape[0] == h_s2t.shape[0] else 0
+    hint = csr.gather_hint() if (part == 0 and ((heads == 1 and D > 32) or (heads == 3 and D <= 4 and table_rows > 0))) else 0
+    rc = lib.bgnn_adaptedconv_aggregate_strided_f32(
         L.ptr_rows(h_t2s), L.ptr_rows(h_s2t), ldh, L.ptr(a_t2s), L.ptr(a_s2t), L.ptr(csr.rowptr), L.ptr(csr.col),
         L.ptr(mask_u8), int(row_begin), row_end, D, float(negative_slope), L.ptr_rows(out), out.stride(0) // heads, L.ptr(alpha),
         L.ptr(ep_scale), L.ptr(ep_shift), 2 if log_softmax else (1 if ep_relu else 0), L.ptr(state_ms), int(part),
         int(row_begin) if park_begin is None else int(park_begin), int(heads), L.ptr(colsum),
-        L.ptr(tq) if not (part == 2 and _P2_STATIC) else None, min(int(h_t2s.shape[0]), int(h_s2t.shape[0])),
-        csr.gather_hint() if (heads == 1 and D > 32 and part == 0) else 0, L.stream())
-    L.check(rc, "bgnn_adaptedconv_aggregate_bounded_f32")
+        L.ptr(tq) if not (part == 2 and _P2_STATIC) else None, table_rows, hint, int(csr.num_edges), int(row_stride), L.stream())
+    L.check(rc, "bgnn_adaptedconv_aggregate_strided_f32")
     return (out, alpha) if want_alpha else out
 
 
diff --git a/include/bgnn.h b/include/bgnn.h
--- a/include/bgnn.h
+++ b/include/bgnn.h
@@ -126,6 +126,16 @@
                                            float* state_ms_opt, int part, int64_t park_begin, int32_t heads, double* colsum_opt,
                                            uint32_t* tile_queue_opt, int64_t table_rows, int32_t gather_hint, void* stream);
 
+int bgnn_adaptedconv_aggregate_strided_f32(const float* h_t2s, const float* h_s2t, int64_t ldh,
+                                           const float* a_t2s, const float* a_s2t,
+                                           const int32_t* rowptr, const int32_t* col, const uint8_t* mask,
+                                           int64_t row_begin, int64_t row_end, int32_t D, float negative_slope,
+                                           float* out, int64_t ldo, float* alpha_opt,
+                                           const float* ep_scale_opt, const float* ep_shift_opt, int ep_relu,
+                                           float* state_ms_opt, int part, int64_t park_begin, int32_t heads, double* colsum_opt,
+                                           uint32_t* tile_queue_opt, int64_t table_rows, int32_t gather_hint,
+                                           int64_t num_edges, int64_t row_stride, void* stream);
+
 size_t bgnn_aggregate_hub_workspace_bytes(int64_t n_segments, int32_t heads, int64_t ldo);
 int bgnn_adaptedconv_aggregate_hub_f32(const float* h_t2s, const float* h_s2t, int64_t ldh,
                                        const float* a_t2s, const float* a_s2t,
@@ -137,6 +147,16 @@
                                        int64_t n_hubs, const int32_t* hub_seg_ptr, const int32_t* seg_bounds,
                                        const int32_t* seg_node, int64_t n_segments, float* alpha_opt,
                                        void* ws, size_t ws_bytes, void* stream);
+int bgnn_adaptedconv_aggregate_hub_strided_f32(const float* h_t2s, const float* h_s2t, int64_t ldh,
+                                               const float* a_t2s, const float* a_s2t,
+                                               const int32_t* rowptr, const int32_t* col, const uint8_t* mask,
+                                               int64_t N, int32_t D, float negative_slope, float* out, int64_t ldo,
+                                               const float* ep_scale_opt, const float* ep_shift_opt, int ep_relu,
+                                               float* state_ms_opt, int32_t heads, double* colsum_opt,
+                                               uint32_t* tile_queue_opt, int32_t hub_threshold, const int32_t* hub_rows,
+                                               int64_t n_hubs, const int32_t* hub_seg_ptr, const int32_t* seg_bounds,
+                                               const int32_t* seg_node, int64_t n_segments, float* alpha_opt,
+                                               void* ws, size_t ws_bytes, int64_t row_stride, void* stream);
 
 int bgnn_adaptedconv_aggregate_bwd_f32(const float* h_t2s, const float* h_s2t, int64_t ldh,
                                        const float* a_t2s, const float* a_s2t,
```
